# PoseLib/PoseLib

Measured on AMD Instinct MI355X. Metric: scored RANSAC hypotheses/sec (P3P@5k corrs, 5pt@5k corrs), higher is better.
Workload: dtype f64; 1 GPU; p3p_5000; correspondences=5000, problems_in_flight_per_gpu=128, distinct_scenes=64

## Files before the change

include/poselib_amd.h:

```cpp
#ifndef POSELIB_AMD_H_
#define POSELIB_AMD_H_
#include <stddef.h>
#include <stdint.h>

#ifdef __cplusplus
extern "C" {
#endif

#define PL_OK 0
#define PL_ERR_NO_DEVICE (-1)
#define PL_ERR_HIP (-2)
#define PL_ERR_INVALID (-3)
#define PL_ERR_UNSUPPORTED (-4)
#define PL_ERR_COMM (-5)

typedef struct {
    uint64_t max_iterations;
    uint64_t min_iterations;
    double dyn_num_trials_mult;
    double success_prob;
    uint64_t seed;
    int32_t progressive_sampling;
    int32_t score_initial_model;
    uint64_t max_prosac_iterations;
// ... 123 lines not shown
} pl_batch_item;
int pl_estimate_batch(pl_batch_item *items, size_t count, int max_in_flight);
int pl_estimate_batch_devices(pl_batch_item *items, size_t count, const int *devices, int num_devices, int max_in_flight);
typedef struct {
    int32_t kind;
    int32_t status;
    pl_device_points a;
    pl_device_points b;
    size_t n;
    const pl_robust_options *opt;
    pl_camera *camera1;
    const pl_camera *camera2;
    void *model;
    uint8_t *inliers;
    pl_ransac_stats *stats;
} pl_batch_item_dev;
int pl_estimate_batch_dev(pl_batch_item_dev *items, size_t count, int max_in_flight);
int pl_debug_point_stats_group_dev(const pl_device_points *x1, const pl_device_points *x2, const size_t *n, size_t count, int centroid,
                                   double *out);
typedef struct {
    const void *data;
    int64_t stride;
    int32_t dtype;
    int32_t reserved;
    double min_score;
} pl_device_scores;
int pl_estimate_dev_scored(int kind, const pl_device_points *a, const pl_device_points *b, const pl_device_scores *scores, size_t n,
                           const pl_robust_options *opt, pl_camera *camera1, const pl_camera *camera2, void *model, uint8_t *inliers,
                           pl_ransac_stats *stats, size_t *n_used);
int pl_estimate_batch_dev_scored(pl_batch_item_dev *items, const pl_device_scores *scores, size_t *n_used, size_t count,
                                 int max_in_flight);
typedef struct {
    uint8_t *data;
    int64_t stride;
} pl_device_mask;
int pl_estimate_dev_masked(int kind, const pl_device_points *a, const pl_device_points *b, const pl_device_scores *scores ,
                           size_t n, const pl_robust_options *opt, pl_camera *camera1, const pl_camera *camera2, void *model,
                           const pl_device_mask *mask, pl_ransac_stats *stats, size_t *n_used);
int pl_estimate_batch_dev_masked(pl_batch_item_dev *items, const pl_device_scores *scores , const pl_device_mask *masks,
                                 size_t *n_used, size_t count, int max_in_flight);
int pl_debug_rank_scores(const pl_device_scores *scores, const size_t *n, size_t count, uint32_t *order, size_t *kept);
int pl_debug_rank_tile(size_t max_n);
typedef struct {
    uint64_t items;
    uint64_t grouped;
    uint64_t focal_grouped;
    uint64_t solo;
    uint64_t fallback;
} pl_batch_report;
void pl_last_batch_report(pl_batch_report *out);

int pl_ransac_pnp(const double *x, const double *X, size_t n, const pl_robust_options *opt, pl_camera_pose *pose,
                  uint8_t *inliers, pl_ransac_stats *stats);
int pl_ransac_pnpf(const double *x, const double *X, size_t n, const pl_robust_options *opt, pl_camera_pose *pose, double *focal,
                   uint8_t *inliers, pl_ransac_stats *stats);
int pl_ransac_relpose(const double *x1, const double *x2, size_t n, const pl_robust_options *opt, pl_camera_pose *pose,
                      uint8_t *inliers, pl_ransac_stats *stats);
int pl_ransac_shared_focal_relpose(const double *x1, const double *x2, size_t n, const pl_robust_options *opt, pl_camera_pose *pose,
                                   double *focal, uint8_t *inliers, pl_ransac_stats *stats);
int pl_refine_shared_focal_relpose(const double *x1, const double *x2, size_t n, const pl_bundle_options *opt, pl_camera_pose *pose,
                                   double *focal, uint32_t *lm_iterations);

int pl_ransac_fundamental(const double *x1, const double *x2, size_t n, const pl_robust_options *opt, double *F,
                          uint8_t *inliers, pl_ransac_stats *stats);
int pl_ransac_homography(const double *x1, const double *x2, size_t n, const pl_robust_options *opt, double *H,
                         uint8_t *inliers, pl_ransac_stats *stats);
int pl_estimate_1D_radial_absolute_pose(const double *points2D, const double *points3D, size_t n, const pl_robust_options *opt,
                                        pl_camera_pose *pose, uint8_t *inliers, pl_ransac_stats *stats);
int pl_ransac_1D_radial_pnp(const double *x, const double *X, size_t n, const pl_robust_options *opt, pl_camera_pose *pose,
                            uint8_t *inliers, pl_ransac_stats *stats);

typedef struct pl_problem pl_problem;
int pl_problem_create(int kind, const double *a, const double *b, size_t n, pl_problem **out);
int pl_problem_create_tangent(const double *x1, const double *x2, size_t n, const pl_camera *camera1, const pl_camera *camera2,
                              pl_problem **out);
int pl_problem_create_dev(int kind, const pl_device_points *a, const pl_device_points *b, size_t n, pl_problem **out);
int pl_problem_create_tangent_dev(const pl_device_points *x1, const pl_device_points *x2, size_t n, const pl_camera *camera1,
                                  const pl_camera *camera2, pl_problem **out);
void pl_problem_destroy(pl_problem *p);
int pl_ransac_run(pl_problem *p, const pl_robust_options *opt, void *model, uint8_t *inliers, pl_ransac_stats *stats);

typedef struct {
    pl_problem *problem;
    const pl_robust_options *opt;
    void *model;
    uint8_t *inliers;
    pl_ransac_stats *stats;
    int32_t status;
    int32_t reserved;
} pl_ransac_item;
int pl_ransac_batch(pl_ransac_item *items, size_t count, int max_in_flight, int group_size);

typedef int (*pl_allgather_fn)(void *user, const void *send, void *recv, size_t bytes);
typedef struct pl_shard {
    int32_t rank, world;
    pl_allgather_fn allgather;
    void *user;
} pl_shard;
int pl_ransac_run_sharded(pl_problem *p, const pl_robust_options *opt, const pl_shard *shard, void *model,
                          uint8_t *inliers, pl_ransac_stats *stats);

int pl_score_model(pl_problem *p, const void *model, double max_error, uint64_t *inlier_count, double *score);
int pl_debug_inlier_mask(pl_problem *p, const void *model, double max_error, uint8_t *mask);
int pl_debug_tangent_chunk(void);
int pl_debug_radial1d_chunk(void);
int pl_debug_group_slices(int kind, uint32_t n_points, uint32_t iterations, uint32_t launch_chunks);
int pl_debug_radial1d_generate(pl_problem *p, const uint32_t *samples, size_t num_iters, uint32_t slots_per_iter, double *models,
                               uint32_t *num_models, uint32_t *totals);
int pl_debug_generate(pl_problem *p, const uint32_t *samples, uint64_t seed, uint64_t pos_base, const uint32_t *positions, size_t num_iters,
                      uint32_t slots_per_iter, int real_focal_check, int route, double *models, uint32_t *num_models, uint32_t *nan_bits,
                      uint32_t *blk_tot, uint32_t *blk_nan, uint32_t *flags);
int pl_debug_score_stream(pl_problem *p, const void *models, size_t n, double max_error, uint32_t *counts,
                          double *scores, int32_t *path_used);
int pl_debug_score_shape(int kind, uint32_t n_points, int matrix_core, int group_form, uint32_t *chunks,
                         uint32_t *points_per_lane);
typedef struct pl_debug_score_member {
    pl_problem *problem;
    const void *models;
    size_t n;
    double max_error;
    uint32_t *counts;
    double *scores;
    uint32_t slices;
    uint32_t slices_used;
    uint32_t chunks;
    int32_t path_used;
} pl_debug_score_member;
int pl_debug_score_stream_ex(int route, pl_debug_score_member *members, size_t num_members, uint32_t *idle_changed);
typedef struct pl_debug_prune_member {
    pl_problem *problem;
    const void *models;
    size_t n;
    double max_error;
    double init_min;
    uint32_t init_max;
    uint32_t cand_cap;
    uint32_t *counts;
    double *scores;
    uint8_t *kept;
    uint32_t *cand;
    uint32_t num_cand;
    uint32_t cstar, chunks, chunk_points;
    uint32_t lead;
    uint32_t lead_max;
    uint32_t num_live, num_selected;
    uint32_t slices, num_preselected;
    double lead_min;
} pl_debug_prune_member;
int pl_debug_score_pruned(int route, pl_debug_prune_member *members, size_t num_members, uint32_t *idle_changed);
int pl_debug_score_survivors(int route, pl_debug_prune_member *members, size_t num_members, uint32_t *const *survivors,
                             uint32_t *idle_changed, uint32_t *guard_changed);
int pl_debug_score_bounded(int route, pl_debug_prune_member *members, size_t num_members, uint32_t *const *bound_counts,
                           double *const *bound_scores, uint8_t *const *tiers, uint32_t *idle_changed, uint32_t *guard_changed);
int pl_debug_score_prune_gate(int kind, uint32_t n_points, uint32_t iterations);
int pl_debug_lm_route(int kind, uint32_t n_points, uint64_t max_iterations, uint32_t *slices);
typedef struct pl_debug_sampler_shape_info {
    uint64_t window;
    uint32_t build, tile;
    uint32_t small_flags, small_doubling, small_segments;
    uint32_t large_flags, large_doubling, large_segments;
} pl_debug_sampler_shape_info;
int pl_debug_sampler_shape(int K, uint64_t N, uint32_t B, uint64_t window, pl_debug_sampler_shape_info *out);
typedef struct pl_debug_sampler_member {
    uint64_t seed, pos_base, N;
    uint32_t B, M;
    const uint8_t *planted;
    uint32_t *positions;
    uint8_t *delta;
    uint64_t *flagbits;
    uint64_t pos_after;
    uint32_t orbit_error, M_used, build_used;
    int32_t delta_guard, ctl_clear, pad;
} pl_debug_sampler_member;
int pl_debug_sample_positions(int route, int K, int build, pl_debug_sampler_member *members, size_t num_members, uint32_t *idle_changed);
int pl_debug_device_math(int fn, const double *x, size_t n, double *out);
int pl_debug_device_math2(int fn, const double *x, const double *y, size_t n, double *out);
int pl_refine_model(pl_problem *p, const pl_bundle_options *opt, const pl_camera *camera, const uint8_t *mask,
                    void *model, uint32_t *lm_iterations);

int pl_bundle_adjust_camera(pl_problem *p, const pl_bundle_options *opt, pl_camera *camera, const uint8_t *mask,
                            pl_camera_pose *pose, uint32_t *lm_iterations);

int pl_p3p(const double *x , const double *X , pl_camera_pose *out );
int pl_p5lp_radial(const double *x , const double *X , pl_camera_pose *out , int *count );
int pl_relpose_5pt(const double *x1 , const double *x2 , pl_camera_pose *out );
int pl_essential_matrix_5pt(const double *x1, const double *x2, double *E );
int pl_relpose_7pt(const double *x1 , const double *x2 , double *F );
int pl_homography_4pt(const double *x1 , const double *x2 , double *H );
int pl_p35pf(const double *x, const double *X, pl_camera_pose *out, double *focals);
int pl_relpose_6pt_shared_focal(const double *x1, const double *x2, pl_camera_pose *out, double *focals);
int pl_solve_focal_batch(int kind, const double *in, size_t count, double *out_models, uint32_t *out_counts);
int pl_solve_batch(int kind, const double *in, size_t count, double *out_models, uint32_t *out_counts);

#ifdef __cplusplus
}
#endif
#endif
```

poselib_amd/_lib.py:

```python
from __future__ import annotations

import ctypes as C
import os
import subprocess

_PKG = os.path.dirname(os.path.abspath(__file__))
_CSRC = os.path.join(_PKG, "csrc")
LIB_PATH = os.path.join(_PKG, "lib", "libposelib_amd.so")
if os.environ.get("POSELIB_AMD_LIB"):
    LIB_PATH = os.environ["POSELIB_AMD_LIB"]

u64, i32, u32, f64 = C.c_uint64, C.c_int32, C.c_uint32, C.c_double

PL_OK, PL_ERR_NO_DEVICE, PL_ERR_HIP, PL_ERR_INVALID, PL_ERR_UNSUPPORTED, PL_ERR_COMM = 0, -1, -2, -3, -4, -5


class RansacOptions(C.Structure):
    _fields_ = [("max_iterations", u64), ("min_iterations", u64), ("dyn_num_trials_mult", f64), ("success_prob", f64),
                ("seed", u64), ("progressive_sampling", i32), ("score_initial_model", i32),
                ("max_prosac_iterations", u64)]


class BundleOptions(C.Structure):
    _fields_ = [("max_iterations", u64), ("loss_type", i32), ("lambda_update", i32), ("damping", i32), ("verbose", i32),
# ... 60 lines not shown
                ("lead_max", u32), ("num_live", u32), ("num_selected", u32), ("slices", u32), ("num_preselected", u32), ("lead_min", f64)]


class DebugSamplerShape(C.Structure):
    _fields_ = [("window", u64), ("build", u32), ("tile", u32), ("small_flags", u32), ("small_doubling", u32), ("small_segments", u32),
                ("large_flags", u32), ("large_doubling", u32), ("large_segments", u32)]


class DebugSamplerMember(C.Structure):
    _fields_ = [("seed", u64), ("pos_base", u64), ("N", u64), ("B", u32), ("M", u32), ("planted", C.c_void_p), ("positions", C.c_void_p),
                ("delta", C.c_void_p), ("flagbits", C.c_void_p), ("pos_after", u64), ("orbit_error", u32), ("M_used", u32),
                ("build_used", u32), ("delta_guard", i32), ("ctl_clear", i32), ("pad", i32)]


PL_F64, PL_F32 = 0, 1


class DevicePoints(C.Structure):
    _fields_ = [("data", C.c_void_p), ("row_stride", C.c_int64), ("dtype", i32), ("cols", i32)]


class BatchItemDev(C.Structure):
    _fields_ = [("kind", i32), ("status", i32), ("a", DevicePoints), ("b", DevicePoints), ("n", C.c_size_t),
                ("opt", C.POINTER(RobustOptions)), ("camera1", C.POINTER(Camera)), ("camera2", C.POINTER(Camera)),
                ("model", C.c_void_p), ("inliers", C.c_void_p), ("stats", C.POINTER(RansacStats))]


class DeviceScores(C.Structure):
    _fields_ = [("data", C.c_void_p), ("stride", C.c_int64), ("dtype", i32), ("reserved", i32), ("min_score", f64)]


class DevicePointsOut(C.Structure):
    _fields_ = [("data", C.c_void_p), ("row_stride", C.c_int64), ("dtype", i32), ("cols", i32)]


class UndistortItemDev(C.Structure):
    _fields_ = [("status", i32), ("reserved", i32), ("camera", C.POINTER(Camera)), ("points2D", DevicePoints), ("n", C.c_size_t),
                ("out", DevicePointsOut)]


class DeviceMask(C.Structure):
    _fields_ = [("data", C.c_void_p), ("stride", C.c_int64)]


class PoseLibAmdError(RuntimeError):
    pass


def build(force: bool = False, verbose: bool = False) -> str:
    srcs = [os.path.join(_CSRC, f) for f in os.listdir(_CSRC) if f.endswith((".h", ".hip", ".cc", ".inc", "Makefile"))]
    srcs.append(os.path.join(os.path.dirname(_PKG), "include", "poselib_amd.h"))
    stale = (not os.path.exists(LIB_PATH)) or any(os.path.getmtime(s) > os.path.getmtime(LIB_PATH) for s in srcs)
    if force or stale:
        cmd = ["make", "-C", _CSRC]
        if not verbose:
            cmd.append("-s")
        subprocess.check_call(cmd)
    return LIB_PATH


_lib = None


def lib():
    global _lib
    if _lib is None:
        if not os.path.exists(LIB_PATH):
            raise PoseLibAmdError(
                f"{LIB_PATH} is missing: build it with `python -c 'import poselib_amd; poselib_amd.build()'` "
                "(there is no CPU fallback)")
        if not os.environ.get("POSELIB_AMD_KEEP_ENV"):
            os.environ.setdefault("GPU_MAX_HW_QUEUES", "16")
        L = C.CDLL(LIB_PATH)
        _declare(L)
        _lib = L
    return _lib


def _declare(L):
    vp, sz, dbl, cint = C.c_void_p, C.c_size_t, C.c_double, C.c_int
    P = C.POINTER
    opt, stats, cam, pose = P(RobustOptions), P(RansacStats), P(Camera), P(CameraPose)
    dpts = P(DevicePoints)
    sig = {
        "pl_default_ransac_options": (None, [P(RansacOptions)]),
        "pl_default_bundle_options": (None, [P(BundleOptions)]),
        "pl_default_robust_options": (None, [opt, cint]),
        "pl_device_count": (cint, []),
        "pl_set_lm_mode": (cint, [cint]),
        "pl_set_device": (cint, [cint]),
        "pl_last_error": (C.c_char_p, []),
        "pl_version": (C.c_char_p, []),
        "pl_abi_version": (cint, []),
        "pl_estimate_absolute_pose": (cint, [vp, vp, sz, opt, cam, pose, vp, stats]),
        "pl_estimate_relative_pose": (cint, [vp, vp, sz, cam, cam, opt, pose, vp, stats]),
        "pl_estimate_fundamental": (cint, [vp, vp, sz, opt, vp, vp, stats]),
        "pl_estimate_homography": (cint, [vp, vp, sz, opt, vp, vp, stats]),
        "pl_estimate_absolute_pose_dev": (cint, [dpts, dpts, sz, opt, cam, pose, vp, stats]),
        "pl_estimate_relative_pose_dev": (cint, [dpts, dpts, sz, cam, cam, opt, pose, vp, stats]),
        "pl_estimate_fundamental_dev": (cint, [dpts, dpts, sz, opt, vp, vp, stats]),
        "pl_estimate_homography_dev": (cint, [dpts, dpts, sz, opt, vp, vp, stats]),
        "pl_problem_create_dev": (cint, [cint, dpts, dpts, sz, P(vp)]),
        "pl_problem_create_tangent_dev": (cint, [dpts, dpts, sz, cam, cam, P(vp)]),
        "pl_debug_check_device_points": (cint, [dpts, sz, cint]),
        "pl_debug_point_stats_dev": (cint, [dpts, dpts, sz, cint, vp]),
        "pl_estimate_batch": (cint, [P(BatchItem), sz, cint]),
        "pl_estimate_batch_devices": (cint, [P(BatchItem), sz, P(C.c_int), cint, cint]),
        "pl_estimate_batch_dev": (cint, [P(BatchItemDev), sz, cint]),
        "pl_debug_point_stats_group_dev": (cint, [dpts, dpts, P(sz), sz, cint, vp]),
        "pl_estimate_dev_scored": (cint, [cint, dpts, dpts, P(DeviceScores), sz, opt, cam, cam, vp, vp, stats, P(sz)]),
        "pl_estimate_batch_dev_scored": (cint, [P(BatchItemDev), P(DeviceScores), P(sz), sz, cint]),
        "pl_estimate_dev_masked": (cint, [cint, dpts, dpts, P(DeviceScores), sz, opt, cam, cam, vp, P(DeviceMask), stats, P(sz)]),
        "pl_estimate_batch_dev_masked": (cint, [P(BatchItemDev), P(DeviceScores), P(DeviceMask), P(sz), sz, cint]),
        "pl_debug_rank_scores": (cint, [P(DeviceScores), P(sz), sz, vp, P(sz)]),
        "pl_debug_rank_tile": (cint, [sz]),
        "pl_last_batch_report": (None, [P(BatchReport)]),
        "pl_ransac_batch": (cint, [P(RansacItem), sz, cint, cint]),
        "pl_undistort_points": (cint, [cam, vp, sz, vp]),
        "pl_undistort_points_dev": (cint, [cam, dpts, sz, P(DevicePointsOut)]),
        "pl_undistort_points_batch_dev": (cint, [P(UndistortItemDev), sz]),
        "pl_ransac_pnp": (cint, [vp, vp, sz, opt, pose, vp, stats]),
        "pl_ransac_pnpf": (cint, [vp, vp, sz, opt, pose, P(dbl), vp, stats]),
        "pl_ransac_relpose": (cint, [vp, vp, sz, opt, pose, vp, stats]),
        "pl_ransac_shared_focal_relpose": (cint, [vp, vp, sz, opt, pose, P(dbl), vp, stats]),
        "pl_solve_focal_batch": (cint, [cint, vp, sz, vp, vp]),
        "pl_p35pf": (cint, [vp, vp, vp, vp]),
        "pl_relpose_6pt_shared_focal": (cint, [vp, vp, vp, vp]),
        "pl_refine_shared_focal_relpose": (cint, [vp, vp, sz, P(BundleOptions), pose, P(dbl), P(C.c_uint32)]),
        "pl_estimate_shared_focal_relative_pose": (cint, [vp, vp, sz, vp, opt, pose, P(dbl), vp, stats]),
        "pl_ransac_fundamental": (cint, [vp, vp, sz, opt, vp, vp, stats]),
        "pl_ransac_homography": (cint, [vp, vp, sz, opt, vp, vp, stats]),
        "pl_problem_create": (cint, [cint, vp, vp, sz, P(vp)]),
        "pl_problem_create_tangent": (cint, [vp, vp, sz, cam, cam, P(vp)]),
        "pl_debug_inlier_mask": (cint, [vp, vp, dbl, vp]),
        "pl_debug_tangent_chunk": (cint, []),
        "pl_debug_radial1d_chunk": (cint, []),
        "pl_debug_group_slices": (cint, [cint, C.c_uint32, C.c_uint32, C.c_uint32]),
        "pl_debug_radial1d_generate": (cint, [vp, vp, sz, C.c_uint32, vp, vp, vp]),
        "pl_debug_generate": (cint, [vp, vp, u64, u64, vp, sz, C.c_uint32, cint, cint, vp, vp, vp, vp, vp, vp]),
        "pl_estimate_1D_radial_absolute_pose": (cint, [vp, vp, sz, opt, pose, vp, stats]),
        "pl_ransac_1D_radial_pnp": (cint, [vp, vp, sz, opt, pose, vp, stats]),
        "pl_p5lp_radial": (cint, [vp, vp, P(CameraPose), P(cint)]),
        "pl_problem_destroy": (None, [vp]),
        "pl_ransac_run": (cint, [vp, opt, vp, vp, stats]),
        "pl_ransac_run_sharded": (cint, [vp, opt, P(Shard), vp, vp, stats]),
        "pl_score_model": (cint, [vp, vp, dbl, P(C.c_uint64), P(dbl)]),
        "pl_debug_score_stream": (cint, [vp, vp, sz, dbl, vp, vp, P(C.c_int32)]),
        "pl_debug_score_shape": (cint, [cint, C.c_uint32, cint, cint, P(C.c_uint32), P(C.c_uint32)]),
        "pl_debug_score_stream_ex": (cint, [cint, P(DebugScoreMember), sz, P(C.c_uint32)]),
        "pl_debug_score_pruned": (cint, [cint, P(DebugPruneMember), sz, P(C.c_uint32)]),
        "pl_debug_score_survivors": (cint, [cint, P(DebugPruneMember), sz, P(C.c_void_p), P(C.c_uint32), P(C.c_uint32)]),
        "pl_debug_score_bounded": (cint, [cint, P(DebugPruneMember), sz, P(C.c_void_p), P(C.c_void_p), P(C.c_void_p), P(C.c_uint32),
                                           P(C.c_uint32)]),
        "pl_debug_score_prune_gate": (cint, [cint, C.c_uint32, C.c_uint32]),
        "pl_debug_lm_route": (cint, [cint, C.c_uint32, u64, P(C.c_uint32)]),
        "pl_debug_sampler_shape": (cint, [cint, u64, C.c_uint32, u64, P(DebugSamplerShape)]),
        "pl_debug_sample_positions": (cint, [cint, cint, cint, P(DebugSamplerMember), sz, P(C.c_uint32)]),
        "pl_debug_device_math": (cint, [cint, vp, sz, vp]),
        "pl_debug_device_math2": (cint, [cint, vp, vp, sz, vp]),
        "pl_refine_model": (cint, [vp, P(BundleOptions), cam, vp, vp, P(C.c_uint32)]),
        "pl_bundle_adjust_camera": (cint, [vp, P(BundleOptions), cam, vp, P(CameraPose), P(C.c_uint32)]),
        "pl_p3p": (cint, [vp, vp, P(CameraPose)]),
        "pl_relpose_5pt": (cint, [vp, vp, P(CameraPose)]),
        "pl_essential_matrix_5pt": (cint, [vp, vp, vp]),
        "pl_relpose_7pt": (cint, [vp, vp, vp]),
        "pl_homography_4pt": (cint, [vp, vp, vp]),
        "pl_solve_batch": (cint, [cint, vp, sz, vp, vp]),
    }
    missing = [name for name in EXPORTED_SYMBOLS if name not in sig]
    assert not missing, f"no signature declared for {missing}"
    for name, (res, args) in sig.items():
        fn = getattr(L, name)
        fn.restype = res
        fn.argtypes = args
    if L.pl_abi_version() != ABI_VERSION:
        raise PoseLibAmdError(f"{LIB_PATH} has record layout version {L.pl_abi_version()}, this binding was written for {ABI_VERSION}: rebuild")


def check(rc: int):
    if rc < 0:
        msg = lib().pl_last_error().decode()
        raise PoseLibAmdError(f"poselib_amd error {rc}: {msg}")
    return rc


ABI_VERSION = 5
EXPORTED_SYMBOLS = [
    "pl_default_ransac_options", "pl_default_bundle_options", "pl_default_robust_options", "pl_device_count",
    "pl_set_device", "pl_last_error", "pl_version", "pl_estimate_absolute_pose", "pl_estimate_relative_pose",
    "pl_estimate_fundamental", "pl_estimate_homography", "pl_ransac_pnp", "pl_ransac_relpose", "pl_ransac_fundamental",
    "pl_ransac_homography", "pl_problem_create", "pl_problem_destroy", "pl_ransac_run", "pl_ransac_run_sharded", "pl_score_model", "pl_debug_score_stream", "pl_refine_model", "pl_bundle_adjust_camera", "pl_p3p", "pl_relpose_5pt",
    "pl_essential_matrix_5pt", "pl_relpose_7pt", "pl_homography_4pt", "pl_solve_batch", "pl_estimate_batch", "pl_estimate_batch_devices", "pl_last_batch_report", "pl_undistort_points",
    "pl_ransac_batch", "pl_debug_device_math", "pl_debug_device_math2", "pl_ransac_pnpf", "pl_ransac_shared_focal_relpose", "pl_refine_shared_focal_relpose",
    "pl_estimate_shared_focal_relative_pose", "pl_solve_focal_batch", "pl_p35pf", "pl_relpose_6pt_shared_focal", "pl_set_lm_mode",
    "pl_abi_version", "pl_problem_create_tangent", "pl_debug_inlier_mask", "pl_debug_tangent_chunk",
    "pl_p5lp_radial", "pl_debug_radial1d_chunk", "pl_debug_radial1d_generate", "pl_debug_group_slices", "pl_debug_generate",
    "pl_debug_score_shape", "pl_debug_score_stream_ex", "pl_debug_score_pruned", "pl_debug_score_survivors", "pl_debug_score_prune_gate",
    "pl_debug_score_bounded", "pl_debug_lm_route",
    "pl_estimate_absolute_pose_dev", "pl_estimate_relative_pose_dev", "pl_estimate_fundamental_dev", "pl_estimate_homography_dev",
    "pl_problem_create_dev", "pl_problem_create_tangent_dev", "pl_debug_check_device_points", "pl_debug_point_stats_dev",
    "pl_debug_sampler_shape", "pl_debug_sample_positions", "pl_estimate_batch_dev", "pl_debug_point_stats_group_dev",
    "pl_estimate_dev_scored", "pl_estimate_batch_dev_scored", "pl_debug_rank_scores", "pl_debug_rank_tile",
    "pl_undistort_points_dev", "pl_undistort_points_batch_dev", "pl_estimate_dev_masked", "pl_estimate_batch_dev_masked",
]
```

poselib_amd/api.py:

```python
from __future__ import annotations

import ctypes as C
import math
import sys
import threading

import numpy as np

from . import _lib as L

LAMBDA_UPDATES = {"NIELSEN": 0, "FIXED_FACTOR": 1}
DAMPINGS = {"LEVENBERG": 0, "MARQUARDT": 1}
LOSS_TYPES = {"TRIVIAL": 0, "TRUNCATED": 1, "HUBER": 2, "CAUCHY": 3, "TRUNCATED_CAUCHY": 4, "TRUNCATED_LE_ZACH": 5}
CAMERA_MODEL_IDS = {"NULL": -1, "SIMPLE_PINHOLE": 0, "PINHOLE": 1, "SIMPLE_RADIAL": 2, "RADIAL": 3, "OPENCV": 4,
                    "OPENCV_FISHEYE": 5, "SIMPLE_RADIAL_FISHEYE": 8, "RADIAL_FISHEYE": 9}
_CAMERA_NAMES = {v: k for k, v in CAMERA_MODEL_IDS.items()}
KIND_ABS, KIND_REL, KIND_FUND, KIND_HOM = 0, 1, 2, 3
KIND_SHARED_FOCAL = 4
KIND_RAD1D = 5
_POSE_KINDS = (KIND_ABS, KIND_REL, KIND_RAD1D)


class CameraPose:

# ... 683 lines not shown
                out.append((_pypose(model), _info(st, inl[: pr.n])))
            else:
                out.append((model.reshape(3, 3).T.copy(), _info(st, inl[: pr.n])))
        return out


def device_math(fn: int, x):
    x = np.ascontiguousarray(x, dtype=np.float64)
    out = np.zeros_like(x)
    L.check(L.lib().pl_debug_device_math(int(fn), _ptr(x), C.c_size_t(x.size), _ptr(out)))
    return out


def device_math2(fn: int, x, y=None):
    x = np.ascontiguousarray(x, dtype=np.float64)
    if y is not None:
        y = np.ascontiguousarray(y, dtype=np.float64)
        if y.shape != x.shape:
            raise ValueError("x and y differ in shape")
    out = np.zeros_like(x)
    L.check(L.lib().pl_debug_device_math2(int(fn), _ptr(x), None if y is None else _ptr(y), C.c_size_t(x.size), _ptr(out)))
    return out


def group_slices(kind: int, n_points: int, iterations: int, launch_chunks: int) -> int:
    return L.check(L.lib().pl_debug_group_slices(int(kind), int(n_points), int(iterations), int(launch_chunks)))


def score_shape(kind: int, n_points: int, matrix_core: bool, group_form: bool):
    chunks, per_lane = C.c_uint32(0), C.c_uint32(0)
    rc = L.lib().pl_debug_score_shape(int(kind), int(n_points), int(bool(matrix_core)), int(bool(group_form)), C.byref(chunks),
                                      C.byref(per_lane))
    if rc == L.PL_ERR_UNSUPPORTED:
        return None
    L.check(rc)
    return chunks.value, per_lane.value


def score_stream_group(members):
    arr = (L.DebugScoreMember * max(len(members), 1))()
    keep = []
    for i, (problem, models, max_error, slices) in enumerate(members):
        n, flat = problem._flat_models(models)
        cnt = np.zeros(max(n, 1), dtype=np.uint32)
        sc = np.zeros(max(n, 1), dtype=np.float64)
        keep.append((n, flat, cnt, sc))
        arr[i] = L.DebugScoreMember(problem._h, _ptr(flat), n, float(max_error), _ptr(cnt), _ptr(sc), int(slices), 0, 0, 0)
    idle = C.c_uint32(0)
    L.check(L.lib().pl_debug_score_stream_ex(2, arr, C.c_size_t(len(members)), C.byref(idle)))
    out = [{"counts": cnt[:n], "scores": sc[:n], "path": arr[i].path_used, "slices": arr[i].slices_used, "chunks": arr[i].chunks}
           for i, (n, _, cnt, sc) in enumerate(keep)]
    return out, idle.value


def sampler_shape(K: int, N: int, B: int, window: int = 0):
    s = L.DebugSamplerShape()
    L.check(L.lib().pl_debug_sampler_shape(int(K), int(N), int(B), int(window), C.byref(s)))
    return {"window": int(s.window), "build": "small" if s.build == 1 else "large", "tile": int(s.tile),
            "small": {"flags": s.small_flags, "doubling": s.small_doubling, "segments": s.small_segments},
            "large": {"flags": s.large_flags, "doubling": s.large_doubling, "segments": s.large_segments}}


_SAMPLER_BUILDS = {None: 0, "small": 1, "large": 2}


def sample_positions(K: int, members, build=None, group: bool = False):
    arr = (L.DebugSamplerMember * max(len(members), 1))()
    keep = []
    for i, m in enumerate(members):
        planted = m.get("planted")
        if planted is not None:
            planted = np.ascontiguousarray(planted, dtype=np.uint8)
            M = int(planted.size)
            if m.get("M", 0) not in (0, M):
                raise ValueError("a planted table has M bytes")
        else:
            M = int(m.get("M", 0)) or sampler_shape(K, m["N"], m["B"])["window"]
        pos = np.zeros(max(int(m["B"]), 1), dtype=np.uint32)
        cap = M if M < (1 << 31) else 0
        delta = np.zeros(cap + 1, dtype=np.uint8)
        bits = np.zeros(cap // 64 + 2, dtype=np.uint64)
        keep.append((planted, pos, delta, bits))
        arr[i] = L.DebugSamplerMember(int(m.get("seed", 0)), int(m.get("pos_base", 0)), int(m["N"]), int(m["B"]), M,
                                      None if planted is None else _ptr(planted), _ptr(pos), _ptr(delta), _ptr(bits))
    idle = C.c_uint32(0)
    L.check(L.lib().pl_debug_sample_positions(2 if group else 0, int(K), _SAMPLER_BUILDS[build], arr, C.c_size_t(len(members)),
                                              C.byref(idle)))
    out = []
    for i, (_, pos, delta, bits) in enumerate(keep):
        a = arr[i]
        words = (a.M_used + 63) // 64
        out.append({"positions": pos, "delta": delta[:a.M_used], "flagbits": bits[:words], "guard": bits[words:a.M_used // 64 + 2],
                    "pos_after": int(a.pos_after), "orbit_error": int(a.orbit_error), "M": int(a.M_used),
                    "build": "small" if a.build_used == 1 else "large", "delta_guard": bool(a.delta_guard),
                    "ctl_clear": bool(a.ctl_clear)})
    return out, idle.value


def score_prune_gate(kind: int, n_points: int, iterations: int) -> bool:
    return bool(L.check(L.lib().pl_debug_score_prune_gate(int(kind), int(n_points), int(iterations))))


def lm_route(kind: int, n_points: int, max_iterations: int = 100):
    slices = C.c_uint32(0)
    return L.check(L.lib().pl_debug_lm_route(int(kind), int(n_points), int(max_iterations), C.byref(slices))), slices.value


def score_pruned(members, route=0):
    arr = (L.DebugPruneMember * max(len(members), 1))()
    keep = []
    cap = 4096
    for i, (problem, models, max_error, init_max, init_min) in enumerate(members):
        n, flat = problem._flat_models(models)
        cnt = np.zeros(max(n, 1), dtype=np.uint32)
        sc = np.zeros(max(n, 1), dtype=np.float64)
        kp = np.zeros(max(n, 1), dtype=np.uint8)
        cand = np.zeros(cap, dtype=np.uint32)
        keep.append((n, flat, cnt, sc, kp, cand))
        arr[i] = L.DebugPruneMember(problem._h, _ptr(flat), n, float(max_error), float(init_min), int(init_max), cap, _ptr(cnt),
                                    _ptr(sc), _ptr(kp), _ptr(cand))
    idle = C.c_uint32(0)
    L.check(L.lib().pl_debug_score_pruned(int(route), arr, C.c_size_t(len(members)), C.byref(idle)))
    out = []
    for i, (n, _, cnt, sc, kp, cand) in enumerate(keep):
        a = arr[i]
        out.append({"counts": cnt[:n], "scores": sc[:n], "kept": kp[:n].astype(bool), "cand": cand[:min(a.num_cand, cap)].copy(),
                    "num_cand": a.num_cand, "cstar": a.cstar, "chunks": a.chunks, "chunk_points": a.chunk_points, "lead": a.lead,
                    "lead_max": a.lead_max, "lead_min": a.lead_min, "num_live": a.num_live, "num_selected": a.num_selected, "num_preselected": a.num_preselected,
                    "slices": a.slices})
    return out, idle.value


def score_survivors(members, route=0):
    arr = (L.DebugPruneMember * max(len(members), 1))()
    outs = (C.c_void_p * max(len(members), 1))()
    keep = []
    for i, (problem, models, max_error) in enumerate(members):
        n, flat = problem._flat_models(models)
        chunks = score_shape(problem.kind, problem.n, True, route == 2)[0]
        sv = np.zeros((chunks, max(n, 1)), dtype=np.uint32)
        keep.append((n, flat, sv))
        arr[i] = L.DebugPruneMember(problem._h, _ptr(flat), n, float(max_error))
        outs[i] = sv.ctypes.data
    idle, guard = C.c_uint32(0), C.c_uint32(0)
    L.check(L.lib().pl_debug_score_survivors(int(route), arr, C.c_size_t(len(members)), outs, C.byref(idle), C.byref(guard)))
    out = []
    for i, (n, _, sv) in enumerate(keep):
        a = arr[i]
        assert a.chunks == sv.shape[0], (a.chunks, sv.shape)
        out.append({"survivors": sv[:, :n], "chunks": a.chunks, "chunk_points": a.chunk_points, "num_live": a.num_live, "slices": a.slices})
    return out, idle.value, guard.value


def score_bounded(members, route=0):
    arr = (L.DebugPruneMember * max(len(members), 1))()
    bcs, bss, trs = ((C.c_void_p * max(len(members), 1))() for _ in range(3))
    keep = []
    cap = 4096
    for i, (problem, models, max_error, init_max, init_min) in enumerate(members):
        n, flat = problem._flat_models(models)
        cnt = np.zeros(max(n, 1), dtype=np.uint32)
        sc = np.zeros(max(n, 1), dtype=np.float64)
        kp = np.zeros(max(n, 1), dtype=np.uint8)
        cand = np.zeros(cap, dtype=np.uint32)
        bc = np.zeros(max(n, 1), dtype=np.uint32)
        bs = np.zeros(max(n, 1), dtype=np.float64)
        tr = np.zeros(max(n, 1), dtype=np.uint8)
        keep.append((n, flat, cnt, sc, kp, cand, bc, bs, tr))
        arr[i] = L.DebugPruneMember(problem._h, _ptr(flat), n, float(max_error), float(init_min), int(init_max), cap, _ptr(cnt),
                                    _ptr(sc), _ptr(kp), _ptr(cand))
        bcs[i], bss[i], trs[i] = bc.ctypes.data, bs.ctypes.data, tr.ctypes.data
    idle, guard = C.c_uint32(0), C.c_uint32(0)
    L.check(L.lib().pl_debug_score_bounded(int(route), arr, C.c_size_t(len(members)), bcs, bss, trs, C.byref(idle), C.byref(guard)))
    out = []
    for i, (n, _, cnt, sc, kp, cand, bc, bs, tr) in enumerate(keep):
        a = arr[i]
        out.append({"counts": cnt[:n], "scores": sc[:n], "kept": kp[:n].astype(bool), "cand": cand[:min(a.num_cand, cap)].copy(),
                    "num_cand": a.num_cand, "cstar": a.cstar, "chunks": a.chunks, "chunk_points": a.chunk_points, "lead": a.lead,
                    "lead_max": a.lead_max, "lead_min": a.lead_min, "num_live": a.num_live, "num_selected": a.num_selected,
                    "num_preselected": a.num_preselected, "slices": a.slices, "bound_counts": bc[:n], "bound_scores": bs[:n],
                    "tiers": tr[:n]})
    return out, idle.value, guard.value


def ransac_batch(problems, opts, max_in_flight=4, group_size=16):
    b = RansacBatch(problems, opts)
    b.run(max_in_flight, group_size)
    return b.results()


def estimate_fundamental(points2D_1, points2D_2, opt=None, initial_F=None, scores=None, min_score=None, inliers_out=None):
    return _estimate_matrix("pl_estimate_fundamental", KIND_FUND, points2D_1, points2D_2, opt, initial_F, scores, min_score, inliers_out)


def estimate_homography(points2D_1, points2D_2, opt=None, initial_H=None, scores=None, min_score=None, inliers_out=None):
    return _estimate_matrix("pl_estimate_homography", KIND_HOM, points2D_1, points2D_2, opt, initial_H, scores, min_score, inliers_out)


def _ransac(fn, kind, a, b, dim_b, opt, initial):
    a, b = _pts(a, 2), _pts(b, dim_b)
    o = _robust_options(opt, kind, initial is not None)
    n = a.shape[0]
    inl = np.zeros(max(n, 1), dtype=np.uint8)
    st = L.RansacStats()
    if kind in _POSE_KINDS:
        pose = _cpose(initial if initial is not None else CameraPose())
        L.check(getattr(L.lib(), fn)(_ptr(a), _ptr(b), C.c_size_t(n), C.byref(o), C.byref(pose), _ptr(inl), C.byref(st)))
        return _pypose(pose), _info(st, inl[:n])
    M = np.ascontiguousarray((np.eye(3) if initial is None else np.asarray(initial, dtype=np.float64)).T.reshape(9))
    L.check(getattr(L.lib(), fn)(_ptr(a), _ptr(b), C.c_size_t(n), C.byref(o), _ptr(M), _ptr(inl), C.byref(st)))
    return M.reshape(3, 3).T.copy(), _info(st, inl[:n])


def ransac_pnp(x, X, opt=None, initial_pose=None):
    return _ransac("pl_ransac_pnp", KIND_ABS, x, X, 3, opt, initial_pose)


def ransac_1D_radial_pnp(x, X, opt=None, initial_pose=None):
    return _ransac("pl_ransac_1D_radial_pnp", KIND_RAD1D, x, X, 3, opt, initial_pose)


def estimate_1D_radial_absolute_pose(points2D, points3D, opt=None, initial_pose=None):
    return _ransac("pl_estimate_1D_radial_absolute_pose", KIND_RAD1D, points2D, points3D, 3, opt, initial_pose)


def ransac_pnpf(x, X, opt=None):
    x, X = _pts(x, 2), _pts(X, 3)
    o = _robust_options(opt, KIND_ABS, False)
    n = x.shape[0]
    inl = np.zeros(max(n, 1), dtype=np.uint8)
    st = L.RansacStats()
    pose = _cpose(CameraPose())
    focal = C.c_double(1.0)
    L.check(L.lib().pl_ransac_pnpf(_ptr(x), _ptr(X), C.c_size_t(n), C.byref(o), C.byref(pose), C.byref(focal), _ptr(inl), C.byref(st)))
    return Image(_pypose(pose), Camera("SIMPLE_PINHOLE", [focal.value, 0.0, 0.0])), _info(st, inl[:n])


class ImagePair:

    def __init__(self, pose=None, camera1=None, camera2=None):
        self.pose = pose or CameraPose()
        self.camera1 = camera1 or Camera("SIMPLE_PINHOLE", [1.0, 0.0, 0.0])
        self.camera2 = camera2 or Camera("SIMPLE_PINHOLE", list(self.camera1.params))


def _shared_focal_pair(pose, focal, pp):
    return ImagePair(_pypose(pose), Camera("SIMPLE_PINHOLE", [focal, pp[0], pp[1]]), Camera("SIMPLE_PINHOLE", [focal, pp[0], pp[1]]))


def ransac_shared_focal_relpose(x1, x2, opt=None, initial_pair=None):
    x1, x2 = _pts(x1, 2), _pts(x2, 2)
    o = _robust_options(opt, KIND_REL, initial_pair is not None)
    n = x1.shape[0]
    inl = np.zeros(max(n, 1), dtype=np.uint8)
    st = L.RansacStats()
    pose = _cpose(initial_pair.pose if initial_pair is not None else CameraPose())
    focal = C.c_double(initial_pair.camera1.focal() if initial_pair is not None else 1.0)
    L.check(L.lib().pl_ransac_shared_focal_relpose(_ptr(x1), _ptr(x2), C.c_size_t(n), C.byref(o), C.byref(pose), C.byref(focal),
                                                   _ptr(inl), C.byref(st)))
    return _shared_focal_pair(pose, focal.value, (0.0, 0.0)), _info(st, inl[:n])


def estimate_shared_focal_relative_pose(points2D_1, points2D_2, pp, opt=None, initial_pair=None):
    x1, x2 = _pts(points2D_1, 2), _pts(points2D_2, 2)
    o = _robust_options(opt, KIND_REL, initial_pair is not None)
    n = x1.shape[0]
    inl = np.zeros(max(n, 1), dtype=np.uint8)
    st = L.RansacStats()
    pose = _cpose(initial_pair.pose if initial_pair is not None else CameraPose())
    focal = C.c_double(initial_pair.camera1.focal() if initial_pair is not None else 1.0)
    ppa = np.ascontiguousarray(pp, dtype=np.float64)
    L.check(L.lib().pl_estimate_shared_focal_relative_pose(_ptr(x1), _ptr(x2), C.c_size_t(n), _ptr(ppa), C.byref(o), C.byref(pose),
                                                           C.byref(focal), _ptr(inl), C.byref(st)))
    return _shared_focal_pair(pose, focal.value, ppa), _info(st, inl[:n])


def refine_shared_focal_relpose(x1, x2, pair, bundle=None):
    x1, x2 = _pts(x1, 2), _pts(x2, 2)
    o = _robust_options({"bundle": bundle or {}}, KIND_REL, False)
    pose = _cpose(pair.pose)
    focal = C.c_double(pair.camera1.focal())
    its = C.c_uint32(0)
    L.check(L.lib().pl_refine_shared_focal_relpose(_ptr(x1), _ptr(x2), C.c_size_t(x1.shape[0]), C.byref(o.bundle), C.byref(pose),
                                                   C.byref(focal), C.byref(its)))
    return _shared_focal_pair(pose, focal.value, (0.0, 0.0)), its.value


def solve_focal_batch(kind, inputs):
    k = {"p35pf": 0, "relpose_6pt_shared_focal": 1}[kind]
    a = np.ascontiguousarray(inputs, dtype=np.float64)
    per, slots = (20, 10) if k == 0 else (36, 60)
    if a.ndim != 2 or a.shape[1] != per:
        raise ValueError(f"expected a (count, {per}) array")
    models = np.zeros((a.shape[0], slots, 8))
    counts = np.zeros(max(a.shape[0], 1), dtype=np.uint32)
    L.check(L.lib().pl_solve_focal_batch(C.c_int(k), _ptr(a), C.c_size_t(a.shape[0]), _ptr(models), _ptr(counts)))
    return models, counts[: a.shape[0]]


def p35pf(x, X):
    models, counts = solve_focal_batch("p35pf", np.r_[_pts(x, 2).reshape(-1), _pts(X, 3).reshape(-1)][None, :])
    return [(CameraPose(m[:4], m[4:7]), float(m[7])) for m in models[0, : counts[0]]]


def relpose_6pt_shared_focal(x1, x2):
    models, counts = solve_focal_batch("relpose_6pt_shared_focal", np.r_[_pts(x1, 3).reshape(-1), _pts(x2, 3).reshape(-1)][None, :])
    return [(CameraPose(m[:4], m[4:7]), float(m[7])) for m in models[0, : counts[0]]]


def ransac_relpose(x1, x2, opt=None, initial_pose=None):
    return _ransac("pl_ransac_relpose", KIND_REL, x1, x2, 2, opt, initial_pose)


def ransac_fundamental(x1, x2, opt=None, initial_F=None):
    return _ransac("pl_ransac_fundamental", KIND_FUND, x1, x2, 2, opt, initial_F)


def ransac_homography(x1, x2, opt=None, initial_H=None):
    return _ransac("pl_ransac_homography", KIND_HOM, x1, x2, 2, opt, initial_H)


class Problem:

    def __init__(self, kind: int, a, b):
        self.kind = kind
        pts = _Points(a, b, 2, 3 if kind in (KIND_ABS, KIND_RAD1D) else 2)
        self.n = pts.n
        self._h = C.c_void_p()
        L.check(pts.fn("pl_problem_create")(kind, pts.a, pts.b, C.c_size_t(self.n), C.byref(self._h)))

    def run(self, opt=None, initial=None):
        o = _robust_options(opt, self.kind, initial is not None)
        inl = np.zeros(max(self.n, 1), dtype=np.uint8)
        st = L.RansacStats()
# ... 413 lines not shown
```

poselib_amd/csrc/driver.cc:

```cpp
#include "../../include/poselib_amd.h"
#include "pl_focal.h"
#include "pl_kernels.h"
#include "pl_ranges.h"
#include "pl_refine_cam.h"
#include "pl_sfocal.h"
#include "pl_solver_6ptf.h"
#include "pl_solver_p35pf.h"
#include "pl_sampler.h"
#include "pl_svd3.h"

#include <algorithm>
#include <atomic>
#include <chrono>
#include <condition_variable>
#include <cmath>
#include <cstdio>
#include <cstdlib>
#include <cstring>
#include <functional>
#include <limits>
#include <mutex>
#include <string>
#include <thread>
#include <vector>
// ... 2453 lines not shown
        return rc;
    bb.nan_bits = nullptr;
    GroupArgs a;
    wire_batch_step(a, run, s, bb);
    rc = debug_score_prepare(c, p, a, bb, z, recs, ident, H);
    if (rc != PL_OK)
        return rc;
    const int path = a.comp.s16.out ? 2 : (run.pf.enabled ? 1 : 0);
    const uint32_t per = (uint32_t)kStreamWaves * 64u / (uint32_t)kScoreThreads;
    const uint32_t slices = slices_in ? slices_in * per : std::max<uint32_t>(1u, std::min<uint32_t>(1536u / s.chunks, H));
    HIP_TRY(launch_score(p->kind, a.score, slices, c->stream));
    HIP_TRY(launch_finalize(a.rec.f, c->stream));
    if (counts)
        HIP_TRY(hipMemcpyAsync(counts, c->count.p, sizeof(uint32_t) * H, hipMemcpyDeviceToHost, c->stream));
    if (scores)
        HIP_TRY(hipMemcpyAsync(scores, c->score.p, sizeof(double) * H, hipMemcpyDeviceToHost, c->stream));
    HIP_TRY(wait_stream(c));
    if (path_used)
        *path_used = path;
    if (slices_used)
        *slices_used = std::max<uint32_t>(1u, slices / per);
    if (chunks_used)
        *chunks_used = chunks;
    return PL_OK;
}
constexpr size_t kDebugScoreMembers = 4;
int debug_score_group(pl_debug_score_member *m, size_t count, uint32_t *idle_changed) {
    if (!m || count == 0 || count > kDebugScoreMembers)
        return fail(PL_ERR_INVALID, "the group form takes 1 .. 4 members");
    for (size_t i = 0; i < count; ++i) {
        if (!m[i].problem || !m[i].models || m[i].n == 0 || m[i].n > (1u << 22) || m[i].problem->n == 0)
            return fail(PL_ERR_INVALID, "member: problem / models missing, no correspondences, or n outside 1 .. 2^22");
        if (m[i].problem->kind != m[0].problem->kind)
            return fail(PL_ERR_INVALID, "the members of a group are of one kind");
    }
    const int kind = m[0].problem->kind;
    if (kind != EST_ABS && kind != EST_REL && kind != EST_FUND && kind != EST_HOM)
        return fail(PL_ERR_INVALID, "tangent and 1D-radial problems have no group form");
    Context *c;
    int rc = get_context(&c);
    if (rc != PL_OK)
        return rc;
    for (size_t i = 0; i < count; ++i)
        if (m[i].problem->device != c->device)
            return fail(PL_ERR_INVALID, "problem lives on another device than the calling thread's");
    struct Slot {
        BatchRun run{};
        BatchShape s{};
        BatchSizes z{};
        BatchBuffers b{};
        size_t bytes = 0;
        char *arena = nullptr;
        ~Slot() {
            if (arena)
                (void)hipFree(arena);
        }
    } slot[1 + kDebugScoreMembers];
    struct Scratch {
        void *p = nullptr;
        ~Scratch() {
            if (p)
                (void)hipFree(p);
        }
    } dtable;
    GroupArgs ha[1 + kDebugScoreMembers];
    GroupDims dims{};
    dims.G = (uint32_t)count + 1;
    dims.P = group_points_per_lane(kind);
    uint32_t launch_chunks = 0;
    for (size_t i = 0; i < count; ++i) {
        Slot &t = slot[i + 1];
        const pl_problem *p = m[i].problem;
        t.run.kind = kind;
        t.run.pts = p->ps;
        t.run.thr2 = m[i].max_error * m[i].max_error;
        t.run.pf = problem_prefilter(p, t.run.thr2);
        t.run.init_max = 0xffffffffu;
        t.s.Bl = (uint32_t)m[i].n, t.s.slots = 1;
        t.s.use_mfma = score_uses_mfma(kind, p->n, t.run.pf);
        t.s.chunks = group_member_chunks(kind, t.s.use_mfma, p->n);
        t.s.point_rows = t.s.chunks * 64u * (uint32_t)dims.P;
        if (m[i].slices > score_slice_limit(kind, t.s.chunks, false))
            return fail(PL_ERR_INVALID, "slices beyond what the scorer's launch takes for this member");
        t.z = batch_step_sizes(kind, t.s);
        if (t.s.use_mfma)
            launch_chunks += t.s.chunks;
    }
    slot[0].run = slot[1].run, slot[0].s = slot[1].s, slot[0].z = slot[1].z;
    for (size_t k = 0; k <= count; ++k) {
        Slot &t = slot[k];
        BatchBuffers unused;
        t.bytes = pack_batch_buffers(nullptr, t.z, unused);
        HIP_TRY(hipMalloc((void **)&t.arena, t.bytes));
        HIP_TRY(hipMemsetAsync(t.arena, k == 0 ? 0xa5 : 0, t.bytes, c->stream));
        pack_batch_buffers(t.arena, t.z, t.b);
        t.b.nan_bits = nullptr;
        t.b.host_meta = nullptr, t.b.host_models = nullptr, t.b.host_ctl = nullptr;
        wire_batch_step(ha[k], t.run, t.s, t.b);
    }
    ha[0].active = 0;
    for (size_t i = 0; i < count; ++i) {
        GroupArgs &a = ha[i + 1];
        const Slot &t = slot[i + 1];
        const uint32_t H = t.s.Bl;
        a.slices = m[i].slices ? m[i].slices
                               : group_score_slices(kind, t.s.use_mfma, group_expected_hypotheses(kind, H, H), H, t.s.chunks, launch_chunks);
        dims.max_B = std::max(dims.max_B, H);
        dims.max_hcap = std::max(dims.max_hcap, a.score.hyp_capacity);
        dims.max_chunks = std::max(dims.max_chunks, a.chunks);
        dims.max_slices = std::max(dims.max_slices, a.slices);
        dims.any_mfma |= a.use_mfma;
        dims.any_queue |= a.use_mfma ? 0u : 1u;
        std::vector<double> recs;
        std::vector<uint32_t> ident(H);
        for (uint32_t k = 0; k < H; ++k)
            ident[k] = k;
        debug_score_records(m[i].problem, m[i].models, H, recs);
        rc = debug_score_prepare(c, m[i].problem, a, t.b, t.z, recs, ident, H);
        if (rc != PL_OK)
            return rc;
        HIP_TRY(hipStreamSynchronize(c->stream));
    }
    ha[0].slices = ha[1].slices;
    HIP_TRY(hipMalloc(&dtable.p, sizeof(GroupArgs) * dims.G));
    HIP_TRY(hipMemcpyAsync(dtable.p, ha, sizeof(GroupArgs) * dims.G, hipMemcpyHostToDevice, c->stream));
    HIP_TRY(launch_group_score(kind, static_cast<const GroupArgs *>(dtable.p), dims, c->stream));
    HIP_TRY(launch_group_finalize_records(static_cast<const GroupArgs *>(dtable.p), dims, c->stream));
    for (size_t i = 0; i < count; ++i) {
        const Slot &t = slot[i + 1];
        if (m[i].counts)
            HIP_TRY(hipMemcpyAsync(m[i].counts, t.b.count, sizeof(uint32_t) * t.s.Bl, hipMemcpyDeviceToHost, c->stream));
        if (m[i].scores)
            HIP_TRY(hipMemcpyAsync(m[i].scores, t.b.score, sizeof(double) * t.s.Bl, hipMemcpyDeviceToHost, c->stream));
    }
    std::vector<uint32_t> idle(slot[0].bytes / 4);
    HIP_TRY(hipMemcpyAsync(idle.data(), slot[0].arena, idle.size() * 4, hipMemcpyDeviceToHost, c->stream));
    HIP_TRY(wait_stream(c));
    uint32_t changed = 0;
    for (uint32_t w : idle)
        changed += w != 0xa5a5a5a5u ? 1u : 0u;
    if (idle_changed)
        *idle_changed = changed;
    for (size_t i = 0; i < count; ++i) {
        m[i].path_used = ha[i + 1].comp.s16.out ? 2 : (slot[i + 1].run.pf.enabled ? 1 : 0);
        m[i].slices_used = ha[i + 1].slices;
        m[i].chunks = ha[i + 1].chunks;
    }
    return PL_OK;
}
struct DebugBoundedOut {
    uint32_t *const *bound_counts;
    double *const *bound_scores;
    uint8_t *const *tiers;
};
int debug_score_pruned(int route, pl_debug_prune_member *m, size_t count, uint32_t *idle_changed, uint32_t *const *survivors = nullptr,
                       uint32_t *guard_changed = nullptr, const DebugBoundedOut *bounded = nullptr) {
    if (route != 0 && route != 2)
        return fail(PL_ERR_INVALID, "route: 0 single launch, 2 group form");
    if (!m || count == 0 || count > (route == 0 ? 1 : kDebugScoreMembers))
        return fail(PL_ERR_INVALID, "the single launch takes one member, the group form 1 .. 4");
    for (size_t i = 0; i < count; ++i) {
        if (!m[i].problem || !m[i].models || m[i].n == 0 || m[i].n > (1u << 22) || m[i].problem->n == 0)
            return fail(PL_ERR_INVALID, "member: problem / models missing, no correspondences, or n outside 1 .. 2^22");
        if (m[i].problem->kind != EST_ABS)
            return fail(PL_ERR_INVALID, "the pruned scorer is the absolute-pose one");
        if (m[i].cand_cap && !m[i].cand)
            return fail(PL_ERR_INVALID, "member: cand_cap without cand");
    }
    Context *c;
    int rc = get_context(&c);
    if (rc != PL_OK)
        return rc;
    for (size_t i = 0; i < count; ++i)
        if (m[i].problem->device != c->device)
            return fail(PL_ERR_INVALID, "problem lives on another device than the calling thread's");
    struct Slot {
        BatchRun run{};
        BatchShape s{};
        BatchSizes z{};
        BatchBuffers b{};
        size_t bytes = 0;
        char *arena = nullptr;
        ~Slot() {
            if (arena)
                (void)hipFree(arena);
        }
    } slot[1 + kDebugScoreMembers];
    struct Scratch {
        void *p = nullptr;
        ~Scratch() {
            if (p)
                (void)hipFree(p);
        }
    } dtable, dbound[kDebugScoreMembers];
    GroupArgs ha[1 + kDebugScoreMembers];
    GroupDims dims{};
    dims.G = (uint32_t)count + 1;
    dims.P = group_points_per_lane(EST_ABS);
    uint32_t launch_chunks = 0;
    for (size_t i = 0; i < count; ++i) {
        Slot &t = slot[i + 1];
        const pl_problem *p = m[i].problem;
        t.run.kind = EST_ABS;
        t.run.pts = p->ps;
        t.run.thr2 = m[i].max_error * m[i].max_error;
        t.run.pf = problem_prefilter(p, t.run.thr2);
        t.run.init_max = m[i].init_max;
        t.run.init_min = m[i].init_min;
        t.s.Bl = (uint32_t)m[i].n, t.s.slots = 1;
        t.s.use_mfma = score_uses_mfma(EST_ABS, p->n, t.run.pf);
        if (!t.s.use_mfma)
            return fail(PL_ERR_UNSUPPORTED, "member: not scored on the matrix cores (size, threshold or coordinates out of range)");
        if (route == 0) {
            t.s.chunks = score_chunks(EST_ABS, p->n, true, true);
            t.s.point_rows = abs16_point_rows(p->n);
        } else {
            t.s.chunks = group_member_chunks(EST_ABS, true, p->n);
            t.s.point_rows = t.s.chunks * 64u * (uint32_t)dims.P;
        }
        t.s.prune = true;
        t.z = batch_step_sizes(EST_ABS, t.s);
        launch_chunks += t.s.chunks;
    }
    slot[0].run = slot[1].run, slot[0].s = slot[1].s, slot[0].z = slot[1].z;
    for (size_t k = (route == 0 ? 1 : 0); k <= count; ++k) {
        Slot &t = slot[k];
        BatchBuffers unused;
        t.bytes = pack_batch_buffers(nullptr, t.z, unused);
        HIP_TRY(hipMalloc((void **)&t.arena, t.bytes));
        HIP_TRY(hipMemsetAsync(t.arena, k == 0 ? 0xa5 : 0, t.bytes, c->stream));
        pack_batch_buffers(t.arena, t.z, t.b);
        t.b.nan_bits = nullptr;
        t.b.host_meta = nullptr, t.b.host_models = nullptr, t.b.host_ctl = nullptr;
        wire_batch_step(ha[k], t.run, t.s, t.b);
        ha[k].score.prune.bound = bounded ? 1u : 0u;
        if (bounded && k > 0) {
            const size_t hcap = ha[k].score.hyp_capacity;
            HIP_TRY(hipMalloc(&dbound[k - 1].p, hcap * 16));
            HIP_TRY(hipMemsetAsync(dbound[k - 1].p, 0xff, hcap * 16, c->stream));
            ha[k].score.prune.bnd_score = static_cast<double *>(dbound[k - 1].p);
            ha[k].score.prune.bnd_count = reinterpret_cast<uint32_t *>(ha[k].score.prune.bnd_score + hcap);
        }
    }
    ha[0].active = 0;
    for (size_t i = 0; i < count; ++i) {
        GroupArgs &a = ha[i + 1];
        const Slot &t = slot[i + 1];
        const uint32_t H = t.s.Bl;
        a.slices = group_score_slices(EST_ABS, true, group_expected_hypotheses(EST_ABS, H, H), H, t.s.chunks, launch_chunks);
        dims.max_B = std::max(dims.max_B, H);
        dims.max_hcap = std::max(dims.max_hcap, a.score.hyp_capacity);
        dims.max_chunks = std::max(dims.max_chunks, a.chunks);
        dims.max_slices = std::max(dims.max_slices, a.slices);
        dims.any_mfma = dims.any_prune = 1;
        dims.any_bound = bounded ? 1u : 0u;
        std::vector<double> recs;
        std::vector<uint32_t> ident(H);
        for (uint32_t k = 0; k < H; ++k)
            ident[k] = k;
        debug_score_records(m[i].problem, m[i].models, H, recs);
        rc = debug_score_prepare(c, m[i].problem, a, t.b, t.z, recs, ident, H);
        if (rc != PL_OK)
            return rc;
        HIP_TRY(hipStreamSynchronize(c->stream));
    }
    uint32_t single_slices = 0;
    if (route == 0) {
        const GroupArgs &a = ha[1];
        const uint32_t slices = std::max<uint32_t>(1u, std::min<uint32_t>(1536u / a.chunks, a.score.hyp_capacity));
        single_slices = std::max<uint32_t>(1u, std::min<uint32_t>(slices * (uint32_t)kScoreThreads / (64u * (uint32_t)kStreamWaves),
                                                                  score_slice_limit(EST_ABS, a.chunks, true)));
        if (survivors) {
            HIP_TRY(launch_score_count(a.score, slices, c->stream));
        } else {
            HIP_TRY(launch_score_pruned(a.score, slices, c->stream));
            if (!bounded)
                HIP_TRY(launch_prune_label(a.score, c->stream));
            HIP_TRY(launch_finalize_records(a.rec, c->stream));
        }
    } else {
        ha[0].slices = ha[1].slices;
        HIP_TRY(hipMalloc(&dtable.p, sizeof(GroupArgs) * dims.G));
        HIP_TRY(hipMemcpyAsync(dtable.p, ha, sizeof(GroupArgs) * dims.G, hipMemcpyHostToDevice, c->stream));
        if (survivors) {
            HIP_TRY(launch_group_score_count(static_cast<const GroupArgs *>(dtable.p), dims, c->stream));
        } else {
            HIP_TRY(launch_group_score(EST_ABS, static_cast<const GroupArgs *>(dtable.p), dims, c->stream));
            for (size_t i = 0; i < count && !bounded; ++i)
                HIP_TRY(launch_prune_label(ha[i + 1].score, c->stream));
            HIP_TRY(launch_group_finalize_records(static_cast<const GroupArgs *>(dtable.p), dims, c->stream));
        }
    }
    std::vector<std::vector<uint32_t>> part(count);
    std::vector<std::vector<uint32_t>> rank(count);
    std::vector<std::vector<uint8_t>> kept(count);
    std::vector<std::vector<RecordMeta>> meta(count);
    std::vector<PruneState> st(count);
    std::vector<BatchCtl> ctl(count);
    std::vector<std::vector<uint32_t>> bcount(count);
    std::vector<std::vector<double>> bscore(count);
    for (size_t i = 0; i < count; ++i) {
        const Slot &t = slot[i + 1];
        const uint32_t H = t.s.Bl;
        if (bounded) {
            const size_t hcap = ha[i + 1].score.hyp_capacity;
            bcount[i].resize(hcap), bscore[i].resize(hcap);
            HIP_TRY(hipMemcpyAsync(bcount[i].data(), ha[i + 1].score.prune.bnd_count, 4 * hcap, hipMemcpyDeviceToHost, c->stream));
            HIP_TRY(hipMemcpyAsync(bscore[i].data(), ha[i + 1].score.prune.bnd_score, 8 * hcap, hipMemcpyDeviceToHost, c->stream));
        }
        if (m[i].counts && !survivors)
            HIP_TRY(hipMemcpyAsync(m[i].counts, t.b.count, sizeof(uint32_t) * H, hipMemcpyDeviceToHost, c->stream));
        if (m[i].scores && !survivors)
            HIP_TRY(hipMemcpyAsync(m[i].scores, t.b.score, sizeof(double) * H, hipMemcpyDeviceToHost, c->stream));
        rank[i].resize(H), kept[i].resize(H), meta[i].resize(kRecordCap);
        HIP_TRY(hipMemcpyAsync(rank[i].data(), t.b.rank, sizeof(uint32_t) * H, hipMemcpyDeviceToHost, c->stream));
        HIP_TRY(hipMemcpyAsync(kept[i].data(), t.b.prune_kept, H, hipMemcpyDeviceToHost, c->stream));
        HIP_TRY(hipMemcpyAsync(meta[i].data(), t.b.rec_meta, sizeof(RecordMeta) * kRecordCap, hipMemcpyDeviceToHost, c->stream));
        HIP_TRY(hipMemcpyAsync(&st[i], t.b.prune_state, sizeof(PruneState), hipMemcpyDeviceToHost, c->stream));
        HIP_TRY(hipMemcpyAsync(&ctl[i], t.b.ctl, sizeof(BatchCtl), hipMemcpyDeviceToHost, c->stream));
        if (survivors || bounded) {
            part[i].resize((size_t)t.s.chunks * ha[i + 1].score.hyp_capacity);
            HIP_TRY(hipMemcpyAsync(part[i].data(), t.b.part_count, sizeof(uint32_t) * part[i].size(), hipMemcpyDeviceToHost, c->stream));
        }
    }
    std::vector<uint32_t> idle(route == 2 ? slot[0].bytes / 4 : 0);
    if (!idle.empty())
        HIP_TRY(hipMemcpyAsync(idle.data(), slot[0].arena, idle.size() * 4, hipMemcpyDeviceToHost, c->stream));
    HIP_TRY(wait_stream(c));
    uint32_t changed = 0;
    for (uint32_t w : idle)
        changed += w != 0xa5a5a5a5u ? 1u : 0u;
    if (idle_changed)
        *idle_changed = changed;
    uint32_t guard = 0;
    for (size_t i = 0; i < count; ++i) {
        const uint32_t H = slot[i + 1].s.Bl, chunks = slot[i + 1].s.chunks;
        m[i].chunks = chunks;
        m[i].chunk_points = slot[i + 1].s.point_rows / chunks;
        m[i].num_live = ctl[i].num_live;
        m[i].slices = route == 0 ? single_slices : ha[i + 1].slices;
        if (survivors) {
            const uint32_t hcap = ha[i + 1].score.hyp_capacity;
            for (uint32_t ch = 0; ch < chunks; ++ch) {
                for (uint32_t k = 0; k < H; ++k)
                    survivors[i][(size_t)ch * H + k] = rank[i][k] == kNoRank ? 0u : part[i][(size_t)ch * hcap + rank[i][k]];
                for (uint32_t p = ctl[i].num_live; p < hcap; ++p)
                    guard += part[i][(size_t)ch * hcap + p] != 0xffffffffu ? 1u : 0u;
            }
            continue;
        }
        if (bounded) {
            const uint32_t hcap = ha[i + 1].score.hyp_capacity;
            for (uint32_t ch = 0; ch < chunks; ++ch)
                for (uint32_t p = ctl[i].num_live; p < hcap; ++p)
                    guard += part[i][(size_t)ch * hcap + p] != 0xffffffffu ? 1u : 0u;
            for (uint32_t k = 0; k < H; ++k) {
                const uint32_t p = rank[i][k];
                const bool live = p != kNoRank;
                const bool has = live && bcount[i][p] != 0xffffffffu;
                bounded->bound_counts[i][k] = has ? bcount[i][p] : 0xffffffffu;
                bounded->bound_scores[i][k] = has ? bscore[i][p] : std::numeric_limits<double>::quiet_NaN();
                bounded->tiers[i][k] = !live ? 3 : kept[i][p] == kKept ? 0 : has ? 2 : 1;
            }
        }
        const bool split = st[i].cstar < chunks;
        uint32_t selected = 0;
        for (uint32_t k = 0; k < H; ++k) {
            const bool live = rank[i][k] != kNoRank;
            const bool kp = !split || !live || kept[i][rank[i][k]] == kKept;
            selected += (split && live && kp) ? 1u : 0u;
            if (m[i].kept)
                m[i].kept[k] = kp ? 1 : 0;
        }
        m[i].num_cand = ctl[i].num_records;
        for (uint32_t r = 0; r < std::min<uint32_t>({ctl[i].num_records, m[i].cand_cap, kRecordCap}); ++r)
            m[i].cand[r] = meta[i][r].k;
        m[i].cstar = st[i].cstar;
        m[i].lead = kPruneLead;
        m[i].lead_max = st[i].lead_max;
        m[i].lead_min = st[i].lead_min;
        m[i].num_selected = selected;
        m[i].num_preselected = st[i].sel_len;
    }
    if (guard_changed)
        *guard_changed = guard;
    return PL_OK;
}
}
int pl_debug_score_pruned(int route, pl_debug_prune_member *members, size_t num_members, uint32_t *idle_changed) {
    if (idle_changed)
        *idle_changed = 0;
    return debug_score_pruned(route, members, num_members, idle_changed);
}
int pl_debug_score_survivors(int route, pl_debug_prune_member *members, size_t num_members, uint32_t *const *survivors,
                             uint32_t *idle_changed, uint32_t *guard_changed) {
    if (idle_changed)
        *idle_changed = 0;
    if (guard_changed)
        *guard_changed = 0;
    if (!survivors)
        return fail(PL_ERR_INVALID, "pl_debug_score_survivors: survivors missing");
    for (size_t i = 0; i < num_members; ++i)
        if (!survivors[i])
            return fail(PL_ERR_INVALID, "pl_debug_score_survivors: a member without an output array");
    return debug_score_pruned(route, members, num_members, idle_changed, survivors, guard_changed);
}
int pl_debug_score_bounded(int route, pl_debug_prune_member *members, size_t num_members, uint32_t *const *bound_counts,
                           double *const *bound_scores, uint8_t *const *tiers, uint32_t *idle_changed, uint32_t *guard_changed) {
    if (idle_changed)
        *idle_changed = 0;
    if (guard_changed)
        *guard_changed = 0;
    if (!bound_counts || !bound_scores || !tiers)
        return fail(PL_ERR_INVALID, "pl_debug_score_bounded: output arrays missing");
    for (size_t i = 0; i < num_members; ++i)
        if (!bound_counts[i] || !bound_scores[i] || !tiers[i])
            return fail(PL_ERR_INVALID, "pl_debug_score_bounded: a member without an output array");
    const DebugBoundedOut out{bound_counts, bound_scores, tiers};
    return debug_score_pruned(route, members, num_members, idle_changed, nullptr, guard_changed, &out);
}
int pl_debug_score_prune_gate(int kind, uint32_t n_points, uint32_t iterations) {
    PrefilterArgs pf{};
    pf.enabled = 1;
    pf.g16 = pf.t16 = pf.h16 = 1.0f, pf.thr = 1.0f;
    if (n_points == 0)
        return fail(PL_ERR_INVALID, "pl_debug_score_prune_gate: n_points > 0");
    const bool mfma = score_uses_mfma(kind, n_points, pf);
    return score_prune_gate(kind, mfma, iterations, kind == EST_ABS ? score_chunks(kind, n_points, true, mfma) : 1u) ? 1 : 0;
}
int pl_debug_lm_route(int kind, uint32_t n_points, uint64_t max_iterations, uint32_t *slices) {
    const bool known = kind == EST_ABS || kind == EST_REL || kind == EST_FUND || kind == EST_HOM || kind == EST_RELT || kind == EST_RAD1D;
    if (!known || n_points == 0 || !slices)
        return fail(PL_ERR_INVALID, "pl_debug_lm_route: kind 0 .. 5, n_points > 0, slices pointer");
    const LMRoute r = lm_route(kind, n_points, true, (uint32_t)std::min<uint64_t>(max_iterations, 0xffffffffu));
    *slices = r.slices;
    return r.kernel;
}
int pl_debug_score_stream(pl_problem *p, const void *models, size_t n, double max_error, uint32_t *counts,
                          double *scores, int32_t *path_used) {
    return debug_score_single(p, models, n, max_error, 0, counts, scores, path_used, nullptr, nullptr);
}
int pl_debug_score_stream_ex(int route, pl_debug_score_member *members, size_t num_members, uint32_t *idle_changed) {
    if (idle_changed)
        *idle_changed = 0;
    if (route != 0 && route != 2)
        return fail(PL_ERR_INVALID, "route: 0 single launch, 2 group form");
    if (route == 2)
        return debug_score_group(members, num_members, idle_changed);
    if (!members || num_members != 1)
        return fail(PL_ERR_INVALID, "the single launch takes one member");
    pl_debug_score_member &m = members[0];
    return debug_score_single(m.problem, m.models, m.n, m.max_error, m.slices, m.counts, m.scores, &m.path_used, &m.slices_used, &m.chunks);
}
int pl_debug_score_shape(int kind, uint32_t n_points, int matrix_core, int group_form, uint32_t *chunks, uint32_t *points_per_lane) {
    const bool four = kind == EST_ABS || kind == EST_REL || kind == EST_FUND || kind == EST_HOM;
    if (!(four || kind == EST_RELT || kind == EST_RAD1D) || n_points == 0 || !chunks || !points_per_lane)
        return fail(PL_ERR_INVALID, "pl_debug_score_shape: kind 0 .. 5, n_points > 0, output pointers");
    if (!four && (matrix_core || group_form))
        return fail(PL_ERR_INVALID, "tangent and 1D-radial problems have neither a matrix-core nor a group form");
    if (matrix_core) {
        PrefilterArgs pf{};
        pf.enabled = 1;
        pf.g16 = pf.t16 = pf.h16 = 1.0f, pf.thr = 1.0f;
        if (!score_uses_mfma(kind, n_points, pf))
            return fail(PL_ERR_UNSUPPORTED, "no problem of this kind and size is scored on the matrix cores");
    }
    if (group_form) {
        *chunks = group_member_chunks(kind, matrix_core != 0, n_points);
        *points_per_lane = (uint32_t)((matrix_core && (kind == EST_REL || kind == EST_FUND)) ? group_mfma2_points_per_lane(kind)
                                                                                           : group_points_per_lane(kind));
    } else {
        *chunks = score_chunks(kind, n_points, true, matrix_core != 0);
        *points_per_lane = (uint32_t)score_points_per_lane(kind, n_points, true, matrix_core != 0);
    }
    return PL_OK;
}

int pl_debug_sampler_shape(int K, uint64_t N, uint32_t B, uint64_t window, pl_debug_sampler_shape_info *out) {
    if ((K != 3 && K != 4 && K != 5 && K != 7) || N < (uint64_t)K || N > 0xffffffffull || B == 0 || !out)
        return fail(PL_ERR_INVALID, "pl_debug_sampler_shape: K in {3, 4, 5, 7}, K <= N < 2^32, B > 0, output pointer");
    const uint64_t M = window ? window : sampler_window((uint32_t)N, K, B);
    const OrbitShape sm = orbit_build_shape(true), lg = orbit_build_shape(false);
    out->window = M;
    out->build = (M <= 0xffffffffull && orbit_small_build((uint32_t)M, N, K)) ? 1u : 2u;
    out->tile = sm.tile;
    out->small_flags = sm.flags, out->small_doubling = sm.doubling, out->small_segments = sm.segments;
    out->large_flags = lg.flags, out->large_doubling = lg.doubling, out->large_segments = lg.segments;
    return PL_OK;
}
int pl_debug_sample_positions(int route, int K, int build, pl_debug_sampler_member *m, size_t count, uint32_t *idle_changed) {
    if (idle_changed)
        *idle_changed = 0;
    if (route != 0 && route != 2)
        return fail(PL_ERR_INVALID, "route: 0 single launches, 2 group form");
    if (build < 0 || build > 2)
        return fail(PL_ERR_INVALID, "build: 0 the launcher's choice, 1 small, 2 large");
    if (K != 3 && K != 4 && K != 5 && K != 7)
        return fail(PL_ERR_INVALID, "K: 3, 4, 5 or 7");
    constexpr size_t kMembers = 4;
    if (!m || count == 0 || count > kMembers)
        return fail(PL_ERR_INVALID, "1 .. 4 members");
    const int kind = K == 3 ? EST_ABS : K == 5 ? EST_REL : K == 7 ? EST_FUND : EST_HOM;
    uint64_t window[kMembers];
    for (size_t i = 0; i < count; ++i) {
        if (m[i].N < (uint64_t)K || m[i].N > 0xffffffffull || m[i].B == 0 || m[i].B > (1u << 20) || !m[i].positions)
            return fail(PL_ERR_INVALID, "member: K <= N < 2^32, B in 1 .. 2^20, positions");
        window[i] = m[i].M ? m[i].M : sampler_window((uint32_t)m[i].N, K, m[i].B);
        if (window[i] > 0x7fffffffull || m[i].pos_base + window[i] >= 0xffffffffull || m[i].pos_base >= 0xffffffffull)
            return fail(PL_ERR_INVALID, "member: a window beyond 2^31 - 1 positions, or one that ends at or beyond draw 2^32 - 1");
        if (route == 2 && (m[i].planted != nullptr) != (m[0].planted != nullptr))
            return fail(PL_ERR_INVALID, "a group is drawn or planted as a whole");
    }
    Context *c;
    int rc = get_context(&c);
    if (rc != PL_OK)
        return rc;
    struct Slot {
        BatchRun run{};
        BatchShape s{};
        BatchSizes z{};
        BatchBuffers b{};
        size_t bytes = 0;
        char *arena = nullptr;
        ~Slot() {
            if (arena)
                (void)hipFree(arena);
        }
    } slot[1 + kMembers];
    struct Scratch {
        void *p = nullptr;
        ~Scratch() {
            if (p)
                (void)hipFree(p);
        }
    } dtable;
    GroupArgs ha[1 + kMembers];
    GroupDims dims{};
    dims.G = (uint32_t)count + 1;
    dims.min_n = 0xffffffffu;
    for (size_t i = 0; i < count; ++i) {
        Slot &t = slot[i + 1];
        t.run.kind = kind;
        t.run.pts.n = (uint32_t)m[i].N;
        t.run.seed = m[i].seed, t.run.pos = m[i].pos_base;
        t.s.B = t.s.Bl = m[i].B, t.s.M = (uint32_t)window[i], t.s.slots = 1, t.s.chunks = 1;
        const BatchSizes full = batch_step_sizes(kind, t.s);
        t.z.positions = full.positions, t.z.delta = full.delta, t.z.flags = full.flags, t.z.ctl = full.ctl;
    }
    slot[0].run = slot[1].run, slot[0].s = slot[1].s, slot[0].z = slot[1].z;
    std::vector<uint64_t> bits;
    for (size_t k = (route == 0 ? 1 : 0); k <= count; ++k) {
        Slot &t = slot[k];
        BatchBuffers unused;
        t.bytes = pack_batch_buffers(nullptr, t.z, unused);
        t.bytes += 256;
        HIP_TRY(hipMalloc((void **)&t.arena, t.bytes));
        HIP_TRY(hipMemsetAsync(t.arena, 0xa5, t.bytes, c->stream));
        pack_batch_buffers(t.arena, t.z, t.b);
        t.b.host_meta = nullptr, t.b.host_models = nullptr, t.b.host_ctl = nullptr;
        wire_batch_step(ha[k], t.run, t.s, t.b);
        if (k == 0)
            continue;
        const pl_debug_sampler_member &mi = m[k - 1];
        group_dims_sampler(dims, t.s.M, t.run.pts.n, t.s.B);
        HIP_TRY(hipMemsetAsync(t.b.positions, 0xff, t.z.positions, c->stream));
        if (mi.planted) {
            const uint32_t M = t.s.M, words = (M + 63u) / 64u;
            bits.assign(words, 0ull);
            for (uint32_t p = 0; p < M; ++p)
                if (mi.planted[p] != (uint8_t)K)
                    bits[p >> 6] |= 1ull << (p & 63u);
// ... 963 lines not shown
```

poselib_amd/csrc/kernels.hip:

```cpp
#include "pl_kernels.h"
#include "pl_global.h"
#include "pl_lm_chain.inc"
#include "pl_device.h"
#include <atomic>
#include "pl_prefilter.h"
#include <cstdlib>
#include "pl_sampler.h"
#include "pl_solver_h4.h"
#include "pl_solver_p3p.h"
#include "pl_solver_p5lp_radial.h"
#include "pl_solver_rel.h"

namespace pl {

typedef const float __attribute__((address_space(4))) *uniform_f32_ptr;
typedef const double __attribute__((address_space(4))) *uniform_f64_ptr;
typedef const uint32_t __attribute__((address_space(4))) *uniform_u32_ptr;
__device__ __forceinline__ uniform_f32_ptr as_uniform(const float *p) { return (uniform_f32_ptr)(uintptr_t)p; }
__device__ __forceinline__ uniform_f64_ptr as_uniform(const double *p) { return (uniform_f64_ptr)(uintptr_t)p; }
__device__ __forceinline__ uniform_u32_ptr as_uniform(const uint32_t *p) { return (uniform_u32_ptr)(uintptr_t)p; }

__device__ __forceinline__ double wave_sum(double v) {
#pragma unroll
    for (int off = 32; off > 0; off >>= 1)
// ... 1043 lines not shown

constexpr int kMfmaQueueCap = 1024;
template <int EST>
__device__ __forceinline__ void mfma_drain(const uint16_t *queue, uint32_t first, uint32_t n0, uint32_t n1, const double *pts, int npw,
                                       const double *__restrict__ models, uint32_t unit_slots, double thr2, double *acc_s,
                                       uint32_t *acc_c) {
    const int lane = threadIdx.x & 63;
    struct Batch {
        uint32_t g;
        bool act;
        double x[EST == EST_ABS ? 5 : 4];
        double M[kModelDoubles];
    };
    auto fetch = [&](uint32_t n, uint32_t at, Batch &b) {
        b.act = (uint32_t)lane < n;
        const uint32_t e = b.act ? (uint32_t)queue[(at + lane) & (kMfmaQueueCap - 1)] : 0xffffu;
        const uint32_t pi = b.act ? (e & 0x1ffu) : 0u;
        b.g = e >> 9;
#pragma unroll
        for (int d = 0; d < (EST == EST_ABS ? 5 : 4); ++d)
            b.x[d] = pts[d * npw + pi];
        const uint32_t slot_g = (uint32_t)__shfl((int)unit_slots, (int)(b.act ? b.g : 0u), 64);
        const double *Mp = models + (size_t)slot_g * kModelStride;
#pragma unroll
        for (int i = 0; i < kModelDoubles; ++i)
            b.M[i] = Mp[i];
    };
    auto finish = [&](const Batch &b) {
        double r2;
        const bool in = eval_point<EST>(b.M, b.x, thr2, r2) && b.act;
        const double v = in ? r2 : 0.0;
        const uint64_t inmask = __builtin_amdgcn_ballot_w64(in);
        const uint32_t g0 = (uint32_t)__builtin_amdgcn_readfirstlane((int)b.g);
        if (inmask && !__builtin_amdgcn_ballot_w64(b.act && b.g != g0)) {
            const double tot = wave_sum_dpp(v);
            if (lane == 0) {
                acc_s[g0] += tot;
                acc_c[g0] += (uint32_t)__popcll(inmask);
            }
        } else if (inmask) {
            add_run_totals(v, inmask, b.g, b.act, lane, acc_s, acc_c);
        }
    };
    __builtin_amdgcn_fence(__ATOMIC_ACQ_REL, "wavefront");
    Batch b0, b1;
    fetch(n0, first, b0);
    if (n1) {
        fetch(n1, first + n0, b1);
        finish(b0);
        finish(b1);
    } else {
        finish(b0);
    }
}

template <int PG>
__device__ __forceinline__ void abs16_tile_bits(const half8_t (&Aop)[kAbs16Dirs], const uint4 (&s_b)[1 + kAbs16Dirs][PG][32], int col, int half,
                                                uint32_t (&out)[16]) {
#pragma unroll
    for (int v = 0; v < 16; ++v)
        out[v] = 0u;
    const float16_t kZero = {0, 0, 0, 0, 0, 0, 0, 0, 0, 0, 0, 0, 0, 0, 0, 0};
    auto products = [&](int g, float16_t &D0, float16_t &D1, float16_t &D2) {
        half8_t Bop[kAbs16Dirs];
#pragma unroll
        for (int d = 0; d < kAbs16Dirs; ++d) {
            const uint4 braw = s_b[half ? 1 + d : 0][g][col];
            __builtin_memcpy(&Bop[d], &braw, 16);
        }
        D0 = __builtin_amdgcn_mfma_f32_32x32x16_f16(Aop[0], Bop[0], kZero, 0, 0, 0);
        D1 = __builtin_amdgcn_mfma_f32_32x32x16_f16(Aop[1], Bop[1], kZero, 0, 0, 0);
        D2 = __builtin_amdgcn_mfma_f32_32x32x16_f16(Aop[2], Bop[2], kZero, 0, 0, 0);
    };
    float16_t D0, D1, D2;
    products(0, D0, D1, D2);
#pragma unroll 16
    for (int g = 1; g < PG; ++g) {
        uint32_t T[16];
#pragma unroll
        for (int v = 0; v < 16; ++v)
            T[v] = __float_as_uint(D0[v]) | __float_as_uint(D1[v]) | __float_as_uint(D2[v]);
        products(g, D0, D1, D2);
#pragma unroll
        for (int v = 0; v < 16; ++v)
            out[v] = __builtin_amdgcn_alignbit(out[v], T[v], 31);
        __builtin_amdgcn_sched_group_barrier(0x002, 16, 0);
        __builtin_amdgcn_sched_group_barrier(0x100, 3, 0);
        __builtin_amdgcn_sched_group_barrier(0x002, 4, 0);
        __builtin_amdgcn_sched_group_barrier(0x008, 1, 0);
        __builtin_amdgcn_sched_group_barrier(0x002, 4, 0);
        __builtin_amdgcn_sched_group_barrier(0x008, 1, 0);
        __builtin_amdgcn_sched_group_barrier(0x002, 4, 0);
        __builtin_amdgcn_sched_group_barrier(0x008, 1, 0);
        __builtin_amdgcn_sched_group_barrier(0x002, 4, 0);
    }
#pragma unroll
    for (int v = 0; v < 16; ++v) {
        const uint32_t sg = __float_as_uint(D0[v]) | __float_as_uint(D1[v]) | __float_as_uint(D2[v]);
        out[v] = __builtin_amdgcn_alignbit(out[v], sg, 31);
    }
}

template <int PG>
__device__ __forceinline__ uint32_t abs16_tile_count_t(const half8_t (&Aop)[kAbs16Dirs], const uint4 (&s_b)[1 + kAbs16Dirs][PG][32], int col,
                                                       int half) {
    static_assert(PG % 2 == 0, "a word holds the 32 pairs of two point groups");
    const float16_t kZero = {0, 0, 0, 0, 0, 0, 0, 0, 0, 0, 0, 0, 0, 0, 0, 0};
    auto products = [&](int g, float16_t &D0, float16_t &D1, float16_t &D2) {
        half8_t Bop[kAbs16Dirs];
#pragma unroll
        for (int d = 0; d < kAbs16Dirs; ++d) {
            const uint4 braw = s_b[half ? 1 + d : 0][g][col];
            __builtin_memcpy(&Bop[d], &braw, 16);
        }
        D0 = __builtin_amdgcn_mfma_f32_32x32x16_f16(Bop[0], Aop[0], kZero, 0, 0, 0);
        D1 = __builtin_amdgcn_mfma_f32_32x32x16_f16(Bop[1], Aop[1], kZero, 0, 0, 0);
        D2 = __builtin_amdgcn_mfma_f32_32x32x16_f16(Bop[2], Aop[2], kZero, 0, 0, 0);
    };
    uint32_t word = 0u, n = 0u;
    float16_t D0, D1, D2;
    products(0, D0, D1, D2);
#pragma unroll 16
    for (int g = 1; g < PG; ++g) {
        uint32_t T[16];
#pragma unroll
        for (int v = 0; v < 16; ++v)
            T[v] = __float_as_uint(D0[v]) | __float_as_uint(D1[v]) | __float_as_uint(D2[v]);
        products(g, D0, D1, D2);
#pragma unroll
        for (int v = 0; v < 16; ++v)
            word = __builtin_amdgcn_alignbit(word, T[v], 31);
        if ((g - 1) % 2)
            n += (uint32_t)__popc(word);
        __builtin_amdgcn_sched_group_barrier(0x002, 16, 0);
        __builtin_amdgcn_sched_group_barrier(0x100, 3, 0);
        __builtin_amdgcn_sched_group_barrier(0x002, 4, 0);
        __builtin_amdgcn_sched_group_barrier(0x008, 1, 0);
        __builtin_amdgcn_sched_group_barrier(0x002, 4, 0);
        __builtin_amdgcn_sched_group_barrier(0x008, 1, 0);
        __builtin_amdgcn_sched_group_barrier(0x002, 4, 0);
        __builtin_amdgcn_sched_group_barrier(0x008, 1, 0);
        __builtin_amdgcn_sched_group_barrier(0x002, 4, 0);
        __builtin_amdgcn_sched_barrier(0);
    }
#pragma unroll
    for (int v = 0; v < 16; ++v) {
        const uint32_t sg = __float_as_uint(D0[v]) | __float_as_uint(D1[v]) | __float_as_uint(D2[v]);
        word = __builtin_amdgcn_alignbit(word, sg, 31);
    }
    n += (uint32_t)__popc(word);
    return 16u * PG - n;
}

constexpr int kScoreAll = 0, kScoreLead = 1, kScoreSel = 2, kScoreCount = 3, kScoreCountAll = 4;
template <int PG, int MODE = kScoreAll>
__device__ __forceinline__ void score_mfma_body(const PointSet &pts, const uint4 *__restrict__ shadow16,
                                                const uint4 *__restrict__ points16,
                                                const double *__restrict__ models, const uint32_t *__restrict__ slots,
                                                const uint32_t *__restrict__ num_hyp_ptr, uint32_t hyp_capacity,
                                                double thr2, uint32_t *__restrict__ part_count,
                                                double *__restrict__ part_score, uint32_t slice, uint32_t chunk,
                                                uint32_t nslices, const uint32_t *__restrict__ sel = nullptr,
                                                uint32_t lead = 0) {
    constexpr int kWaves = kMfmaThreads / 64;
    constexpr int NPW = 32 * PG;
    __shared__ double s_pts[5][NPW];
    __shared__ uint16_t s_queue[kWaves][kMfmaQueueCap];
    __shared__ double s_acc_s[kWaves][64];
    __shared__ uint32_t s_acc_c[kWaves][64];
    __shared__ uint32_t s_next_unit;
    __shared__ uint4 s_b[1 + kAbs16Dirs][PG][32];
    const int lane = threadIdx.x & 63;
    const int wave = __builtin_amdgcn_readfirstlane((int)(threadIdx.x >> 6));
    const int col = lane & 31, half = lane >> 5;

    const uint32_t H = MODE == kScoreLead ? min(*as_uniform(num_hyp_ptr), lead) : *as_uniform(num_hyp_ptr);
    const uint32_t waves_per_chunk = nslices * kWaves;
    {
        uint32_t kb0, gn0;
        if (!unit_of_ticket<32u>(slice * kWaves, H, waves_per_chunk, kb0, gn0))
            return;
    }

    uint32_t validbits = 0;
#pragma unroll
    for (int g = 0; g < PG; ++g)
        validbits |= (chunk * NPW + g * 32 + col < pts.n) ? (1u << (PG - 1 - g)) : 0u;
    const uint4 *const prow = points16 + (size_t)chunk * NPW * 4;
    for (uint32_t j = threadIdx.x; j < (uint32_t)NPW; j += kMfmaThreads) {
        const uint32_t i = chunk * NPW + j;
        const uint32_t ic = i < pts.n ? i : 0u;
#pragma unroll
        for (int d = 0; d < 5; ++d)
            s_pts[d][j] = pts.a[d][ic];
#pragma unroll
        for (int r = 0; r < 1 + kAbs16Dirs; ++r)
            s_b[r][j >> 5][j & 31] = prow[(size_t)j * 4 + r];
    }
    if (threadIdx.x == 0)
        s_next_unit = 0;
    __syncthreads();

    uint16_t *const queue = s_queue[wave];
    double *const acc_s = s_acc_s[wave];
    uint32_t *const acc_c = s_acc_c[wave];
    auto request_ticket = [&]() -> uint32_t {
        uint32_t t = 0;
        if (lane == 0) {
            const uint32_t k = atomicAdd(&s_next_unit, 1u);
            t = slice * kWaves + (k % kWaves) + (k / kWaves) * waves_per_chunk;
        }
        return t;
    };
    uint32_t ticket = (uint32_t)__builtin_amdgcn_readfirstlane((int)request_ticket());
    uint32_t kb, gn;
    while (unit_of_ticket<32u>(ticket, H, waves_per_chunk, kb, gn)) {
        const uint32_t pending = request_ticket();
        uint32_t unit_pos = 0;
        if constexpr (MODE == kScoreSel)
            unit_pos = sel ? sel[kb + min((uint32_t)lane, gn - 1u)] : kb + min((uint32_t)lane, gn - 1u);
        const uint32_t unit_slots = slots[MODE == kScoreSel ? unit_pos : kb + min((uint32_t)lane, gn - 1u)];
        acc_s[lane] = 0.0;
        acc_c[lane] = 0;
        uint32_t qhead = 0, qtail = 0;

        auto drain_pair = [&](uint32_t n2) {
            mfma_drain<EST_ABS>(queue, qhead, 64u, n2, &s_pts[0][0], NPW, models, unit_slots, thr2, acc_s, acc_c);
            qhead += 64u + n2;
        };
        auto drain = [&](uint32_t n) {
            mfma_drain<EST_ABS>(queue, qhead, n, 0u, &s_pts[0][0], NPW, models, unit_slots, thr2, acc_s, acc_c);
            qhead += n;
        };

        const uint32_t ngroups32 = (gn + 31u) / 32u;
        auto load_a = [&](uint32_t hg, uint4 (&A)[kAbs16Dirs]) {
            const uint4 *row = shadow16 + (size_t)(kb + 32u * hg + (uint32_t)col) * 4;
            if constexpr (MODE == kScoreSel)
                row = shadow16 + (size_t)(uint32_t)__shfl((int)unit_pos, (int)(32u * hg + (uint32_t)col), 64) * 4;
#pragma unroll
            for (int d = 0; d < kAbs16Dirs; ++d)
                A[d] = row[half ? 3 : d];
        };
        uint4 Araw[kAbs16Dirs];
        load_a(0, Araw);
        for (uint32_t hg = 0; hg < ngroups32; ++hg) {
            half8_t Aop[kAbs16Dirs];
#pragma unroll
            for (int d = 0; d < kAbs16Dirs; ++d)
                __builtin_memcpy(&Aop[d], &Araw[d], 16);
            if (hg + 1 < ngroups32)
                load_a(hg + 1, Araw);
            uint32_t out[16];
            abs16_tile_bits<PG>(Aop, s_b, col, half, out);
            const bool partial_group = hg * 32u + 32u > gn;
            auto expand_round = [&](int v, bool check_slot) {
                const uint32_t slot = hg * 32u + 8u * (uint32_t)(v >> 2) + 4u * (uint32_t)half + (uint32_t)(v & 3);
                uint32_t bits = ~out[v] & validbits;
                if (check_slot && slot >= gn)
                    bits = 0u;
                const uint64_t anyb = __builtin_amdgcn_ballot_w64(bits != 0u);
                if (anyb) {
                    const uint32_t cnt = (uint32_t)__popc(bits);
                    if (!__builtin_amdgcn_ballot_w64(cnt > 1u)) {
                        const uint32_t below = __builtin_amdgcn_mbcnt_hi((uint32_t)(anyb >> 32), __builtin_amdgcn_mbcnt_lo((uint32_t)anyb, 0u));
                        if (bits) {
                            const uint32_t g = (uint32_t)(PG - 1 - (31 - __clz((int)bits)));
                            queue[(qtail + below) & (kMfmaQueueCap - 1)] = (uint16_t)((slot << 9) | (g * 32u + (uint32_t)col));
                        }
                        qtail += (uint32_t)__popcll(anyb);
                    } else {
                        const uint32_t incl = wave_scan_u32(cnt);
                        const uint32_t total = (uint32_t)__builtin_amdgcn_readlane((int)incl, 63);
                        uint32_t pos = qtail + incl - cnt;
                        uint32_t rest = bits;
                        while (rest) {
                            const int hi = 31 - __clz((int)rest);
                            rest &= ~(1u << hi);
                            const uint32_t g = (uint32_t)(PG - 1 - hi);
                            queue[pos & (kMfmaQueueCap - 1)] = (uint16_t)((slot << 9) | (g * 32u + (uint32_t)col));
                            ++pos;
                        }
                        qtail += total;
                    }
                    while (qtail - qhead >= 128u)
                        drain_pair(64u);
                }
            };
            if (partial_group) {
#pragma unroll
                for (int v = 0; v < 16; ++v)
                    expand_round(v, true);
            } else {
#pragma unroll
                for (int v = 0; v < 16; ++v)
                    expand_round(v, false);
            }
        }
        if (qtail - qhead > 64u)
            drain_pair(qtail - qhead - 64u);
        else if (qtail != qhead)
            drain(qtail - qhead);
        __builtin_amdgcn_fence(__ATOMIC_ACQ_REL, "wavefront");
        if ((uint32_t)lane < gn) {
            const size_t o = MODE == kScoreSel ? (size_t)chunk * hyp_capacity + unit_pos : (size_t)chunk * hyp_capacity + kb + lane;
            part_score[o] = acc_s[lane];
            part_count[o] = acc_c[lane];
        }
        ticket = (uint32_t)__builtin_amdgcn_readfirstlane((int)pending);
    }
}

template <int PG>
__device__ __forceinline__ void score_count_body(uint32_t n_points, const uint4 *__restrict__ shadow16, const uint4 *__restrict__ points16,
                                                 const uint32_t *__restrict__ num_hyp_ptr, uint32_t hyp_capacity,
                                                 uint32_t *__restrict__ survivors, uint32_t slice, uint32_t chunk, uint32_t nslices,
                                                 uint32_t first) {
    constexpr int kWaves = kMfmaThreads / 64;
    constexpr int NPW = 32 * PG;
    __shared__ uint4 s_b[1 + kAbs16Dirs][PG][32];
    __shared__ uint32_t s_next_unit;
    const int lane = threadIdx.x & 63;
    const int col = lane & 31, half = lane >> 5;
    const uint32_t Hall = *as_uniform(num_hyp_ptr);
    if (Hall <= first)
        return;
    const uint32_t H = Hall - first;
    const uint32_t waves_per_chunk = nslices * kWaves;
    {
        uint32_t kb0, gn0;
        if (!unit_of_ticket<32u>(slice * kWaves, H, waves_per_chunk, kb0, gn0))
            return;
    }
    const uint32_t pad = chunk * NPW + NPW > n_points ? chunk * NPW + NPW - n_points : 0u;
    const uint4 *const prow = points16 + (size_t)chunk * NPW * 4;
    for (uint32_t j = threadIdx.x; j < (uint32_t)NPW; j += kMfmaThreads) {
#pragma unroll
        for (int r = 0; r < 1 + kAbs16Dirs; ++r)
            s_b[r][j >> 5][j & 31] = prow[(size_t)j * 4 + r];
    }
    if (threadIdx.x == 0)
        s_next_unit = 0;
    __syncthreads();

    auto request_ticket = [&]() -> uint32_t {
        uint32_t t = 0;
        if (lane == 0) {
            const uint32_t k = atomicAdd(&s_next_unit, 1u);
            t = slice * kWaves + (k % kWaves) + (k / kWaves) * waves_per_chunk;
        }
        return t;
    };
    uint32_t ticket = (uint32_t)__builtin_amdgcn_readfirstlane((int)request_ticket());
    uint32_t kb, gn;
    while (unit_of_ticket<32u>(ticket, H, waves_per_chunk, kb, gn)) {
        const uint32_t pending = request_ticket();
        const uint32_t ngroups32 = (gn + 31u) / 32u;
        auto load_a = [&](uint32_t hg, uint4 (&A)[kAbs16Dirs]) {
            const uint4 *row = shadow16 + (size_t)min(first + kb + 32u * hg + (uint32_t)col, Hall - 1u) * 4;
#pragma unroll
            for (int d = 0; d < kAbs16Dirs; ++d)
                A[d] = row[half ? 3 : d];
        };
        uint4 Araw[kAbs16Dirs];
        load_a(0, Araw);
        for (uint32_t hg = 0; hg < ngroups32; ++hg) {
            half8_t Aop[kAbs16Dirs];
#pragma unroll
            for (int d = 0; d < kAbs16Dirs; ++d)
                __builtin_memcpy(&Aop[d], &Araw[d], 16);
            if (hg + 1 < ngroups32)
                load_a(hg + 1, Araw);
            const uint32_t mine = abs16_tile_count_t<PG>(Aop, s_b, col, half);
            const auto both = __builtin_amdgcn_permlane32_swap(mine, mine, false, false);
            uint32_t total = both[0] + both[1];
            if (pad)
                total = max(total, pad) - pad;
            if (half == 0 && 32u * hg + (uint32_t)col < gn)
                survivors[(size_t)chunk * hyp_capacity + first + kb + 32u * hg + (uint32_t)col] = total;
        }
        ticket = (uint32_t)__builtin_amdgcn_readfirstlane((int)pending);
    }
}

template <int PG>
__global__ __launch_bounds__(kMfmaThreads) __attribute__((amdgpu_waves_per_eu(4, 8))) void k_score_mfma(PointSet pts, const uint4 *__restrict__ shadow16,
                                                               const uint4 *__restrict__ points16,
                                                               const double *__restrict__ models,
                                                               const uint32_t *__restrict__ slots,
                                                               const uint32_t *__restrict__ num_hyp_ptr,
                                                               uint32_t hyp_capacity, double thr2,
                                                               uint32_t *__restrict__ part_count,
                                                               double *__restrict__ part_score,
                                                               uint32_t *__restrict__ tickets) {
    (void)tickets;
    uint32_t slice, chunk;
    slice_chunk_of_workgroup(gridDim.x, gridDim.y, slice, chunk);
    score_mfma_body<PG>(pts, shadow16, points16, models, slots, num_hyp_ptr, hyp_capacity, thr2, part_count, part_score, slice,
                        chunk, gridDim.x);
}
template <int PG>
__global__ __launch_bounds__(kMfmaThreads) __attribute__((amdgpu_waves_per_eu(4, 8))) void k_score_mfma_g(const GroupArgs *ga) {
    const GroupArgs &g = ga[blockIdx.z];
    uint32_t slice, chunk;
    if (!g.active || !g.use_mfma || !slice_chunk_of_workgroup(g.slices, g.chunks, slice, chunk))
        return;
    const ScoreArgs a = globalised(g.score);
    score_mfma_body<PG>(a.pts, static_cast<const uint4 *>(a.shadow16), static_cast<const uint4 *>(a.points16), a.models, a.slots,
                        a.num_hyp, a.hyp_capacity, a.thr2, a.part_count, a.part_score, slice, chunk, g.slices);
}
template <int MODE> __host__ __device__ constexpr uint32_t pruned_slices(uint32_t slices) {
    return MODE == kScoreLead ? (slices < 2u ? slices : 2u) : MODE == kScoreSel ? (slices + 3u) / 4u : slices;
}
template <int PG, int MODE> __device__ __forceinline__ void score_mfma_pruned(const ScoreArgs &a, uint32_t slice, uint32_t chunk, uint32_t nslices) {
    static_assert(MODE == kScoreLead || MODE == kScoreSel || MODE == kScoreCount || MODE == kScoreCountAll, "the plain launch is k_score_mfma's");
    const PruneArgs &pr = a.prune;
    if (!pr.st && MODE != kScoreSel)
        return;
    if constexpr (MODE == kScoreCountAll) {
        score_count_body<PG>(a.pts.n, static_cast<const uint4 *>(a.shadow16), static_cast<const uint4 *>(a.points16), a.num_hyp,
                             a.hyp_capacity, a.part_count, slice, chunk, nslices, 0u);
    } else if constexpr (MODE == kScoreCount) {
        const uint32_t cstar = *as_uniform(&pr.st->cstar);
        if (cstar >= pr.chunks || chunk >= cstar)
            return;
        score_count_body<PG>(a.pts.n, static_cast<const uint4 *>(a.shadow16), static_cast<const uint4 *>(a.points16), a.num_hyp,
                             a.hyp_capacity, a.part_count, slice, chunk, nslices, pr.lead);
    } else {
        const uint32_t *len = MODE == kScoreSel && pr.st ? &pr.st->sel_len : a.num_hyp;
        score_mfma_body<PG, MODE>(a.pts, static_cast<const uint4 *>(a.shadow16), static_cast<const uint4 *>(a.points16), a.models, a.slots,
                                  len, a.hyp_capacity, a.thr2, a.part_count, a.part_score, slice, chunk, nslices, pr.st ? pr.sel : nullptr,
                                  pr.lead);
    }
}
template <int PG, int MODE>
__global__ __launch_bounds__(kMfmaThreads) __attribute__((amdgpu_waves_per_eu(4, 8))) void k_score_mfma_pr(ScoreArgs a) {
    uint32_t slice, chunk;
    slice_chunk_of_workgroup(gridDim.x, gridDim.y, slice, chunk);
    score_mfma_pruned<PG, MODE>(a, slice, chunk, gridDim.x);
}
template <int PG, int MODE>
__global__ __launch_bounds__(kMfmaThreads) __attribute__((amdgpu_waves_per_eu(4, 8))) void k_score_mfma_pr_g(const GroupArgs *ga) {
    const GroupArgs &g = ga[blockIdx.z];
    uint32_t slice, chunk;
    const uint32_t ns = pruned_slices<MODE>(g.slices);
    if (!g.active || !g.use_mfma || !slice_chunk_of_workgroup(ns, g.chunks, slice, chunk))
        return;
    score_mfma_pruned<PG, MODE>(globalised(g.score), slice, chunk, ns);
}

__device__ __forceinline__ void prune_lead_body(const ScoreArgs &a) {
    __shared__ uint32_t wmax[4];
    __shared__ double wmin[4];
    const PruneArgs &pr = a.prune;
    const uint32_t n = min(*a.num_hyp, pr.lead), N = a.pts.n;
    uint32_t bmax = 0;
    double bmin = 1.7976931348623157e308;
    for (uint32_t p = threadIdx.x; p < n; p += 256) {
        uint32_t c = 0;
        double s = 0.0;
        for (uint32_t ch = 0; ch < pr.chunks; ++ch) {
            c += a.part_count[(size_t)ch * a.hyp_capacity + p];
            s += a.part_score[(size_t)ch * a.hyp_capacity + p];
        }
        bmax = max(bmax, c);
        bmin = fmin(bmin, s + (double)(N - c) * a.thr2);
    }
#pragma unroll
    for (int off = 32; off > 0; off >>= 1) {
        bmax = max(bmax, (uint32_t)__shfl_xor(bmax, off, 64));
        bmin = fmin(bmin, __shfl_xor(bmin, off, 64));
    }
    if ((threadIdx.x & 63) == 0) {
        wmax[threadIdx.x >> 6] = bmax;
        wmin[threadIdx.x >> 6] = bmin;
    }
    __syncthreads();
    if (threadIdx.x == 0) {
        uint32_t lmax = pr.init_max;
        double lmin = pr.init_min;
        for (int w = 0; w < 4; ++w) {
            lmax = max(lmax, wmax[w]);
            lmin = fmin(lmin, wmin[w]);
        }
        const double need = fmax(lmin / a.thr2, (double)(N - min(lmax, N))) + (double)kPruneMargin;
        uint32_t cstar = pr.chunks;
        if (need < (double)N)
            cstar = (uint32_t)ceil(need / (double)pr.chunk_points);
        pr.st->lead_max = lmax;
        pr.st->lead_min = lmin;
        pr.st->cstar = max(1u, min(cstar, pr.chunks));
        pr.st->sel_len = 0;
        pr.st->pad = 0;
    }
}
__global__ __launch_bounds__(256) void k_prune_lead(ScoreArgs a) { prune_lead_body(a); }
__global__ __launch_bounds__(256) void k_prune_lead_g(const GroupArgs *ga) {
    const GroupArgs &g = ga[blockIdx.z];
    if (!g.active || !g.use_mfma || !g.score.prune.st)
        return;
    prune_lead_body(globalised(g.score));
}

__device__ __forceinline__ bool prune_rule(uint32_t cs, double sum, uint32_t S, uint32_t N, double thr2, const PruneState &st) {
    return cs + (N - S) <= st.lead_max && sum + (double)(S - cs) * thr2 > st.lead_min * (1.0 + kPruneScoreMargin);
}
__device__ __forceinline__ uint32_t prune_keeps(const ScoreArgs &a, uint32_t p, uint32_t H, uint32_t cstar) {
    const PruneArgs &pr = a.prune;
    if (p >= H)
        return 0u;
    if (p < pr.lead || cstar >= pr.chunks)
        return 1u;
    const uint32_t N = a.pts.n, S = min(cstar * pr.chunk_points, N);
    uint32_t cs = 0;
    for (uint32_t ch = 0; ch < cstar; ++ch)
        cs += a.part_count[(size_t)ch * a.hyp_capacity + p];
    return prune_rule(cs, 0.0, S, N, a.thr2, *pr.st) ? 0u : 1u;
}
__global__ __launch_bounds__(256) void k_prune_label(ScoreArgs a) {
    const PruneArgs &pr = a.prune;
    const uint32_t H = *a.num_hyp, cstar = pr.st->cstar, p = blockIdx.x * 256u + threadIdx.x;
    if (p >= H || p < pr.lead || cstar >= pr.chunks || pr.kept[p] != kKept)
        return;
    const uint32_t N = a.pts.n, S = min(cstar * pr.chunk_points, N);
    uint32_t cs = 0;
    double sum = 0.0;
    for (uint32_t ch = 0; ch < cstar; ++ch) {
        cs += a.part_count[(size_t)ch * a.hyp_capacity + p];
        sum += a.part_score[(size_t)ch * a.hyp_capacity + p];
    }
    if (prune_rule(cs, sum, S, N, a.thr2, *pr.st))
        pr.kept[p] = kPrunedExact;
}
__device__ __forceinline__ void prune_flags_body(const ScoreArgs &a) {
    __shared__ uint32_t wt[16];
    const PruneArgs &pr = a.prune;
    const uint32_t H = *a.num_hyp, cstar = pr.st->cstar;
    if (blockIdx.x * 1024u >= H)
        return;
    const uint32_t p = blockIdx.x * 1024u + threadIdx.x;
    const uint32_t keep = prune_keeps(a, p, H, cstar);
    if (p < H)
        pr.kept[p] = (uint8_t)keep;
    const uint32_t tot = wave_sum_u32(keep);
    if ((threadIdx.x & 63) == 0)
        wt[threadIdx.x >> 6] = tot;
    __syncthreads();
    if (threadIdx.x == 0) {
        uint32_t t = 0;
        for (int w = 0; w < 16; ++w)
            t += wt[w];
        pr.blk_kept[blockIdx.x] = t;
    }
}
__device__ __forceinline__ void prune_list_body(const ScoreArgs &a) {
    __shared__ uint32_t wt[16], wb[16];
    const PruneArgs &pr = a.prune;
    const uint32_t H = *a.num_hyp;
    if (blockIdx.x * 1024u >= H)
        return;
    const int lane = threadIdx.x & 63, wave = threadIdx.x >> 6;
    uint32_t before = 0;
    for (uint32_t j = threadIdx.x; j < blockIdx.x; j += 1024u)
        before += pr.blk_kept[j];
    before = wave_sum_u32(before);
    const uint32_t p = blockIdx.x * 1024u + threadIdx.x;
    const uint32_t keep = p < H ? (uint32_t)pr.kept[p] : 0u;
    const uint32_t inc = wave_scan_u32(keep);
    if (lane == 63)
        wt[wave] = inc;
    if (lane == 0)
        wb[wave] = before;
    __syncthreads();
    uint32_t at = inc - keep;
    for (int w = 0; w < 16; ++w)
        at += wb[w] + (w < wave ? wt[w] : 0u);
    if (keep)
        pr.sel[at] = p;
    if (p == H - 1u)
        pr.st->sel_len = at + keep;
}
__global__ __launch_bounds__(1024) void k_prune_flags(ScoreArgs a) { prune_flags_body(a); }
__global__ __launch_bounds__(1024) void k_prune_list(ScoreArgs a) { prune_list_body(a); }
__global__ __launch_bounds__(1024) void k_prune_flags_g(const GroupArgs *ga) {
    const GroupArgs &g = ga[blockIdx.z];
    if (!g.active || !g.use_mfma || !g.score.prune.st)
        return;
    prune_flags_body(globalised(g.score));
}
__global__ __launch_bounds__(1024) void k_prune_list_g(const GroupArgs *ga) {
    const GroupArgs &g = ga[blockIdx.z];
    if (!g.active || !g.use_mfma || !g.score.prune.st)
        return;
    prune_list_body(globalised(g.score));
}

constexpr int kBoundThreads = 512;
constexpr uint32_t kBoundGroups = 16;
template <int P> __device__ __forceinline__ void score_bound_body(const ScoreArgs &a, uint32_t wg, uint32_t nwg) {
    constexpr int kWaves = kBoundThreads / 64;
    constexpr uint32_t NPW = 64u * P;
    __shared__ uint32_t s_c[kWaves][64];
    __shared__ uint64_t s_q[kWaves][64];
    __shared__ uint32_t s_und[64];
    __shared__ uint32_t s_nund;
    const PruneArgs &pr = a.prune;
    if (!pr.st || !pr.bound || *as_uniform(&pr.st->cstar) >= pr.chunks)
        return;
    const uint32_t first = min(*as_uniform(a.num_hyp), pr.lead), len = *as_uniform(&pr.st->sel_len);
    if (len <= first || (uint64_t)wg * 64u >= len - first)
        return;
    const int lane = threadIdx.x & 63;
    const int wave = __builtin_amdgcn_readfirstlane((int)(threadIdx.x >> 6));
    const PrefilterArgs pf = a.pf;
    const uint32_t chunks = pr.chunks;
    const bool resident = chunks <= (uint32_t)kWaves;
    float x[P], y[P], X[P], Y[P], Z[P], fw[P];
    bool valid[P];
    uint64_t vmask[P];
    auto load_chunk = [&](uint32_t chunk) {
#pragma unroll
        for (int p = 0; p < P; ++p) {
            const uint32_t i = chunk * NPW + (uint32_t)p * 64u + (uint32_t)lane;
            valid[p] = i < a.pts.n;
            vmask[p] = __builtin_amdgcn_ballot_w64(valid[p]);
            const uint32_t ic = valid[p] ? i : 0u;
            const double Xd = a.pts.a[2][ic], Yd = a.pts.a[3][ic], Zd = a.pts.a[4][ic];
            x[p] = (float)a.pts.a[0][ic], y[p] = (float)a.pts.a[1][ic];
            X[p] = (float)Xd, Y[p] = (float)Yd, Z[p] = (float)Zd;
            fw[p] = pf_point_abs(Xd, Yd, Zd, pf.gx);
        }
    };
    load_chunk(min((uint32_t)wave, chunks - 1u));
    const uint32_t lead_max = pr.st->lead_max;
    const double beat = pr.st->lead_min * (1.0 + kPruneScoreMargin);
    auto decide = [&](uint32_t pos) -> bool {
        uint32_t c = 0;
        uint64_t q = 0;
#pragma unroll
        for (int w = 0; w < kWaves; ++w) {
            c += s_c[w][lane];
            q += s_q[w][lane];
        }
        const double qd = (double)q * 9.5367431640625e-07;
        double s_lb = a.thr2 * qd;
        if (fma(a.thr2, qd, -s_lb) < 0.0)
            s_lb = __longlong_as_double(__double_as_longlong(s_lb) - 1);
        const bool keep = !(c <= lead_max && s_lb > beat);
        if (!keep)
            pr.kept[pos] = kDropped;
        if (pr.bnd_count)
            pr.bnd_count[pos] = c, pr.bnd_score[pos] = s_lb;
        return keep;
    };
    const uint32_t nent = len - first;
    for (uint32_t u = wg; (uint64_t)u * 64u < nent; u += nwg) {
        const uint32_t e = first + u * 64u + (uint32_t)lane;
        const uint32_t pos = pr.sel[min(e, len - 1u)];
        const float4 *sh = reinterpret_cast<const float4 *>(a.models + (size_t)a.slots[pos] * kModelStride + kShadowOff);
        float4 rv[4];
#pragma unroll
        for (int k = 0; k < 4; ++k)
            rv[k] = sh[k];
        const uint32_t n = min(64u, nent - u * 64u);
        auto model_of_lane = [&](uint32_t j, float (&r)[16]) {
#pragma unroll
            for (int k = 0; k < 4; ++k) {
                r[4 * k + 0] = __builtin_bit_cast(float, __builtin_amdgcn_readlane(__builtin_bit_cast(int, rv[k].x), (int)j));
                r[4 * k + 1] = __builtin_bit_cast(float, __builtin_amdgcn_readlane(__builtin_bit_cast(int, rv[k].y), (int)j));
                r[4 * k + 2] = __builtin_bit_cast(float, __builtin_amdgcn_readlane(__builtin_bit_cast(int, rv[k].z), (int)j));
                r[4 * k + 3] = __builtin_bit_cast(float, __builtin_amdgcn_readlane(__builtin_bit_cast(int, rv[k].w), (int)j));
            }
        };
        uint32_t my_c = 0;
        uint64_t my_q = 0;
        for (uint32_t ch = (uint32_t)wave; ch < chunks; ch += (uint32_t)kWaves) {
            if (!resident)
                load_chunk(ch);
            for (uint32_t j = 0; j < n; ++j) {
                float r[16];
                model_of_lane(j, r);
                const float gt = pf_abs_bound_slack(r, pf.gx);
                uint32_t c = 0, q = 0;
#pragma unroll
                for (int p = 0; p + 1 < P; p += 2) {
                    const v2f Xp = {X[p], X[p + 1]}, Yp = {Y[p], Y[p + 1]}, Zp = {Z[p], Z[p + 1]};
                    const v2f xp = {x[p], x[p + 1]}, yp = {y[p], y[p + 1]}, w = {fw[p], fw[p + 1]};
                    const v2f z0 = pk_fma(bc(r[0]), Xp, pk_fma(bc(r[1]), Yp, pk_fma(bc(r[2]), Zp, bc(r[9]))));
                    const v2f z1 = pk_fma(bc(r[3]), Xp, pk_fma(bc(r[4]), Yp, pk_fma(bc(r[5]), Zp, bc(r[10]))));
                    const v2f z2 = pk_fma(bc(r[6]), Xp, pk_fma(bc(r[7]), Yp, pk_fma(bc(r[8]), Zp, bc(r[11]))));
                    const v2f a0 = pk_fma(-xp, z2, z0);
                    const v2f a1 = pk_fma(-yp, z2, z1);
                    const v2f W = w + bc(gt);
                    const v2f B = pk_fma(bc(pf.thr), z2, W);
#pragma unroll
                    for (int e2 = 0; e2 < 2; ++e2) {
                        const uint64_t out = vmask[p + e2] & (__builtin_amdgcn_ballot_w64(fmaxf(fabsf(a0[e2]), fabsf(a1[e2])) > B[e2]) |
                                                              __builtin_amdgcn_ballot_w64(z2[e2] < -W[e2]));
                        q += (uint32_t)__popcll(out);
                        c += (uint32_t)__popcll(vmask[p + e2] & ~out);
                    }
                }
                if constexpr (P & 1) {
                    constexpr int p = P - 1;
                    const uint64_t out = vmask[p] & __builtin_amdgcn_ballot_w64(pf_abs_outlier(r, gt, pf.thr, x[p], y[p], X[p], Y[p], Z[p], fw[p]));
                    q += (uint32_t)__popcll(out);
                    c += (uint32_t)__popcll(vmask[p] & ~out);
                }
                if ((uint32_t)lane == j)
                    my_c += c, my_q += q;
            }
        }
        s_c[wave][lane] = my_c;
        s_q[wave][lane] = my_q << 20;
        __syncthreads();
        bool open = false;
        if (wave == 0) {
            open = (uint32_t)lane < n && decide(pos);
            const uint64_t und = __builtin_amdgcn_ballot_w64(open);
            if (open)
                s_und[__builtin_amdgcn_mbcnt_hi((uint32_t)(und >> 32), __builtin_amdgcn_mbcnt_lo((uint32_t)und, 0u))] = (uint32_t)lane;
            if (lane == 0)
                s_nund = (uint32_t)__popcll(und);
        }
        __syncthreads();
        const uint32_t nund = (uint32_t)__builtin_amdgcn_readfirstlane((int)s_nund);
        if (nund) {
            my_c = 0, my_q = 0;
            for (uint32_t ch = (uint32_t)wave; ch < chunks; ch += (uint32_t)kWaves) {
                if (!resident)
                    load_chunk(ch);
                for (uint32_t k = 0; k < nund; ++k) {
                    const uint32_t j = (uint32_t)__builtin_amdgcn_readfirstlane((int)s_und[k]);
                    float r[16];
                    model_of_lane(j, r);
                    const float gt = pf_abs_bound_slack(r, pf.gx);
                    uint32_t c = 0, q = 0;
#pragma unroll
                    for (int p = 0; p < P; ++p) {
                        const float L = pf_abs_r2_lower(r, gt, x[p], y[p], X[p], Y[p], Z[p], fw[p]);
                        c += (uint32_t)__popcll(__builtin_amdgcn_ballot_w64(valid[p] && L < pf.thr2_up));
                        q += valid[p] ? pf_bound_quantum(L, pf.inv_thr2_dn) : 0u;
                    }
                    q = (uint32_t)__builtin_amdgcn_readlane((int)wave_scan_u32(q), 63);
                    if ((uint32_t)lane == j)
                        my_c += c, my_q += q;
                }
            }
            s_c[wave][lane] = my_c;
            s_q[wave][lane] = my_q;
            __syncthreads();
            if (open)
                (void)decide(pos);
        }
        __syncthreads();
    }
}
template <int P> __global__ __launch_bounds__(kBoundThreads) void k_score_bound(ScoreArgs a) { score_bound_body<P>(a, blockIdx.x, gridDim.x); }
__global__ __launch_bounds__(kBoundThreads) void k_score_bound_g(const GroupArgs *ga) {
    const GroupArgs &g = ga[blockIdx.z];
    if (!g.active || !g.use_mfma || !g.score.prune.st)
        return;
    score_bound_body<5>(globalised(g.score), blockIdx.x, gridDim.x);
}
__device__ __forceinline__ void prune_bound_body(const ScoreArgs &a) {
    __shared__ uint32_t wt[16];
    const PruneArgs &pr = a.prune;
    if (!pr.bound || pr.st->cstar >= pr.chunks)
        return;
    const uint32_t first = min(*a.num_hyp, pr.lead), len = pr.st->sel_len;
    const int lane = threadIdx.x & 63, wave = threadIdx.x >> 6;
    uint32_t base = 0;
    __syncthreads();
    for (uint32_t t0 = first; t0 < len; t0 += 1024u) {
        const uint32_t e = t0 + threadIdx.x;
        uint32_t keep = 0, p = 0;
        if (e < len) {
            p = pr.sel[e];
            keep = pr.kept[p] != kDropped ? 1u : 0u;
        }
        const uint32_t inc = wave_scan_u32(keep);
        if (lane == 63)
            wt[wave] = inc;
        __syncthreads();
        uint32_t at = base + inc - keep, tot = 0;
        for (int w = 0; w < 16; ++w) {
            at += w < wave ? wt[w] : 0u;
            tot += wt[w];
        }
        if (keep)
            pr.sel[at] = p;
        base += tot;
        __syncthreads();
    }
    if (threadIdx.x == 0)
        pr.st->sel_len = base;
}
__global__ __launch_bounds__(1024) void k_prune_bound(ScoreArgs a) { prune_bound_body(a); }
__global__ __launch_bounds__(1024) void k_prune_bound_g(const GroupArgs *ga) {
    const GroupArgs &g = ga[blockIdx.z];
    if (!g.active || !g.use_mfma || !g.score.prune.st)
        return;
    prune_bound_body(globalised(g.score));
}



template <int EST, int PG>
__device__ __forceinline__ void score_mfma2_body(const PointSet &pts, const uint4 *__restrict__ hypop,
                                                 const double *__restrict__ models, const uint32_t *__restrict__ slots,
                                                 const uint32_t *__restrict__ num_hyp_ptr, uint32_t hyp_capacity,
                                                 double thr2, const PrefilterArgs &pf, uint32_t *__restrict__ part_count,
                                                 double *__restrict__ part_score, uint32_t slice, uint32_t chunk,
                                                 uint32_t nslices) {
    static_assert(EST == EST_REL || EST == EST_FUND, "Sampson scores");
    constexpr int kWaves = kMfmaThreads / 64;
    constexpr int NPW = 32 * PG;
    constexpr int NBR = (EST == EST_REL) ? 6 : 1;
    __shared__ double s_pts[4][NPW];
    __shared__ double s_bear[NBR][(EST == EST_REL) ? NPW : 1];
    __shared__ uint16_t s_queue[kWaves][kMfmaQueueCap];
    __shared__ double s_acc_s[kWaves][64];
    __shared__ uint32_t s_acc_c[kWaves][64];
    __shared__ uint32_t s_next_unit;
    __shared__ uint4 s_bop[PG][3][64];
    const int lane = threadIdx.x & 63;
    const int wave = __builtin_amdgcn_readfirstlane((int)(threadIdx.x >> 6));
    const int col = lane & 31, half = lane >> 5;

    for (uint32_t j = threadIdx.x; j < (uint32_t)NPW; j += kMfmaThreads) {
        const uint32_t i = chunk * NPW + j;
        const uint32_t ic = i < pts.n ? i : 0u;
        const double a0 = pts.a[0][ic], a1 = pts.a[1][ic], b0 = pts.a[2][ic], b1 = pts.a[3][ic];
        s_pts[0][j] = a0, s_pts[1][j] = a1, s_pts[2][j] = b0, s_pts[3][j] = b1;
        if constexpr (EST == EST_REL) {
            const Vec3 u1 = bearing(a0, a1), u2 = bearing(b0, b1);
            s_bear[0][j] = u1.x, s_bear[1][j] = u1.y, s_bear[2][j] = u1.z;
            s_bear[3][j] = u2.x, s_bear[4][j] = u2.y, s_bear[5][j] = u2.z;
        }
    }
    uint32_t validbits = 0;
#pragma unroll
    for (int g = 0; g < PG; ++g)
        validbits |= (chunk * NPW + g * 32 + col < pts.n) ? (1u << (PG - 1 - g)) : 0u;
    for (uint32_t j = threadIdx.x; j < (uint32_t)NPW; j += kMfmaThreads) {
        const uint32_t i = chunk * NPW + j;
        const bool valid = i < pts.n;
        const uint32_t ic = valid ? i : 0u;
        Sampson16Operand o;
        pf16_sampson_point(pts.a[0][ic], pts.a[1][ic], pts.a[2][ic], pts.a[3][ic], valid, pf.t16, o);
#pragma unroll
        for (int b = 0; b < 6; ++b) {
            const uint16_t *h = b < 4 ? o.c + 8 * b : o.s + 8 * (b - 4);
            s_bop[j >> 5][b >> 1][(j & 31) + 32 * (b & 1)] =
                make_uint4((uint32_t)h[0] | ((uint32_t)h[1] << 16), (uint32_t)h[2] | ((uint32_t)h[3] << 16),
                           (uint32_t)h[4] | ((uint32_t)h[5] << 16), (uint32_t)h[6] | ((uint32_t)h[7] << 16));
        }
    }
    if (threadIdx.x == 0)
        s_next_unit = 0;
    __syncthreads();

    const uint32_t H = *as_uniform(num_hyp_ptr);
    const float t16 = pf.t16;
    uint16_t *const queue = s_queue[wave];
    double *const acc_s = s_acc_s[wave];
    uint32_t *const acc_c = s_acc_c[wave];
    const uint32_t waves_per_chunk = nslices * kWaves;
    auto request_ticket = [&]() -> uint32_t {
        uint32_t t = 0;
        if (lane == 0) {
            const uint32_t k = atomicAdd(&s_next_unit, 1u);
            t = slice * kWaves + (k % kWaves) + (k / kWaves) * waves_per_chunk;
        }
        return t;
    };
    uint32_t ticket = (uint32_t)__builtin_amdgcn_readfirstlane((int)request_ticket());
    uint32_t kb, gn;
    while (unit_of_ticket(ticket, H, waves_per_chunk, kb, gn)) {
        const uint32_t pending = request_ticket();
        const uint32_t unit_slots = slots[kb + min((uint32_t)lane, gn - 1u)];
        acc_s[lane] = 0.0;
        acc_c[lane] = 0;
        uint32_t qhead = 0, qtail = 0;

        auto drain = [&](uint32_t n) {
            __builtin_amdgcn_fence(__ATOMIC_ACQ_REL, "wavefront");
            const bool act = (uint32_t)lane < n;
            const uint32_t e = act ? (uint32_t)queue[(qhead + lane) & (kMfmaQueueCap - 1)] : 0xffffu;
            const uint32_t g = e >> 9, pi = act ? (e & 0x1ffu) : 0u;
            const double x0 = s_pts[0][pi], x1 = s_pts[1][pi], x2 = s_pts[2][pi], x3 = s_pts[3][pi];
            const double *Mp = models + (size_t)(uint32_t)__shfl((int)unit_slots, (int)(act ? g : 0u), 64) * kModelStride;
            double M[kModelDoubles];
#pragma unroll
            for (int i = 0; i < kModelDoubles; ++i)
                M[i] = Mp[i];
            double r2 = sampson_sq(M + kMatOff, x0, x1, x2, x3);
            bool in = r2 < thr2;
            if constexpr (EST == EST_REL) {
                if (in) {
                    Quat q;
                    q.w = M[0], q.x = M[1], q.y = M[2], q.z = M[3];
                    in = check_cheirality(q, v3(M[4], M[5], M[6]), v3(s_bear[0][pi], s_bear[1][pi], s_bear[2][pi]),
                                          v3(s_bear[3][pi], s_bear[4][pi], s_bear[5][pi]), 0.01);
                }
            }
// ... 1859 lines not shown
}

static uint32_t xcd_slices(uint32_t s) { return std::max<uint32_t>(1u, s); }

template <int E>
static hipError_t launch_score_est(const ScoreArgs &a, uint32_t slices, hipStream_t stream) {
    uint32_t chunks;
    int P;
    const PrefilterArgs pf = a.pf;
    const bool streaming = (a.shadow && a.compact64) || a.shadow16;
    score_shape(E, a.pts.n, streaming, a.shadow16 != nullptr, chunks, P);
    if constexpr (E == EST_REL || E == EST_FUND) {
        if (streaming && a.shadow16) {
            const uint32_t mslices = std::min<uint32_t>(slices * (uint32_t)kScoreThreads / (uint32_t)kMfmaThreads,
                                                        score_slice_limit(E, chunks, true));
            const dim3 mgrid(xcd_slices(mslices), chunks);
            const dim3 mblock(kMfmaThreads);
#define PL_M2_CASE(PP)                                                                                                 \
    case PP:                                                                                                           \
        k_score_mfma2<E, 2 * PP><<<mgrid, mblock, 0, stream>>>(a.pts, static_cast<const uint4 *>(a.shadow16), a.models, \
                                                              a.slots, a.num_hyp, a.hyp_capacity, a.thr2, pf,          \
                                                              a.part_count, a.part_score);                             \
        break;
            switch (P) {
                PL_M2_CASE(1)
                PL_M2_CASE(2)
                PL_M2_CASE(3)
                PL_M2_CASE(4)
                PL_M2_CASE(5)
                PL_M2_CASE(6)
            default:
                return hipErrorInvalidValue;
            }
#undef PL_M2_CASE
            return hipGetLastError();
        }
    }
    if constexpr (E == EST_HOM) {
        if (streaming && a.shadow16) {
            const dim3 mgrid(xcd_slices(slices * (uint32_t)kScoreThreads / (uint32_t)kMfmaThreads), chunks);
            const dim3 mblock(kMfmaThreads);
#define PL_MH_CASE(PP)                                                                                                 \
    case PP:                                                                                                           \
        k_score_mfmah<2 * PP><<<mgrid, mblock, 0, stream>>>(a.pts, static_cast<const uint4 *>(a.shadow16), a.models,    \
                                                          a.slots, a.num_hyp, a.hyp_capacity, a.thr2, pf, a.part_count, \
                                                          a.part_score);                                                \
        break;
            switch (P) {
                PL_MH_CASE(1)
                PL_MH_CASE(2)
                PL_MH_CASE(3)
                PL_MH_CASE(4)
                PL_MH_CASE(5)
            default:
                return hipErrorInvalidValue;
            }
#undef PL_MH_CASE
            return hipGetLastError();
        }
    }
    if constexpr (E == EST_ABS) {
        if (streaming && a.shadow16) {
            const uint32_t mslices = std::min<uint32_t>(slices * (uint32_t)kScoreThreads / (uint32_t)kMfmaThreads,
                                                        score_slice_limit(E, chunks, true));
            const dim3 mgrid(xcd_slices(mslices), chunks);
            const dim3 mblock(kMfmaThreads);
            if (!a.points16)
                return hipErrorInvalidValue;
#define PL_M_CASE(PP)                                                                                                  \
    case PP:                                                                                                           \
        k_score_mfma<2 * PP><<<mgrid, mblock, 0, stream>>>(a.pts, static_cast<const uint4 *>(a.shadow16),                \
                                                         static_cast<const uint4 *>(a.points16), a.models, a.slots,    \
                                                         a.num_hyp, a.hyp_capacity, a.thr2, a.part_count, a.part_score, \
                                                         a.tickets);                                                   \
        break;
            switch (P) {
                PL_M_CASE(1)
                PL_M_CASE(2)
                PL_M_CASE(3)
                PL_M_CASE(4)
                PL_M_CASE(5)
            default:
                return hipErrorInvalidValue;
            }
#undef PL_M_CASE
            return hipGetLastError();
        }
    }
    if (streaming) {
        const dim3 qgrid(std::max<uint32_t>(1u, slices * (uint32_t)kScoreThreads / (uint32_t)kQueueThreads), chunks);
        const dim3 qblock(kQueueThreads);
#define PL_Q_CASE(PP)                                                                                                  \
    case PP:                                                                                                           \
        k_score_queue<E, PP><<<qgrid, qblock, 0, stream>>>(a.pts, a.shadow, a.compact64, a.num_hyp, a.hyp_capacity,      \
                                                         a.thr2, pf, a.part_count, a.part_score, a.tickets);           \
        break;
        switch (P) {
            PL_Q_CASE(1)
            PL_Q_CASE(2)
            PL_Q_CASE(3)
            PL_Q_CASE(4)
            PL_Q_CASE(5)
            PL_Q_CASE(6)
        default:
            return hipErrorInvalidValue;
        }
#undef PL_Q_CASE
        return hipGetLastError();
    }
    return hipErrorInvalidValue;
}

hipError_t launch_score_seq(int est, const SeqScoreArgs &a, hipStream_t stream) {
    if (a.cap == 0)
        return hipSuccess;
    const dim3 grid(std::min<uint32_t>(a.cap, 128u)), block(kSeqThreads);
    PL_DISPATCH_EST_0TO5(est, k_score_seq<E><<<grid, block, 0, stream>>>(a));
    return hipGetLastError();
}
int tangent_score_chunk() { return kTangentChunk; }
int radial1d_score_chunk() { return kRadialChunk; }
hipError_t launch_prune_lead(const ScoreArgs &a, hipStream_t stream) {
    k_prune_lead<<<dim3(1), dim3(256), 0, stream>>>(a);
    return hipGetLastError();
}
hipError_t launch_prune_select(const ScoreArgs &a, hipStream_t stream) {
    const uint32_t nb = std::max<uint32_t>(1u, (a.hyp_capacity + 1023u) / 1024u);
    k_prune_flags<<<dim3(nb), dim3(1024), 0, stream>>>(a);
    k_prune_list<<<dim3(nb), dim3(1024), 0, stream>>>(a);
    return hipGetLastError();
}
hipError_t launch_group_prune_lead(const GroupArgs *args, const GroupDims &d, hipStream_t stream) {
    k_prune_lead_g<<<dim3(1, 1, d.G), dim3(256), 0, stream>>>(args);
    return hipGetLastError();
}
hipError_t launch_group_prune_select(const GroupArgs *args, const GroupDims &d, hipStream_t stream) {
    const uint32_t nb = std::max<uint32_t>(1u, (d.max_hcap + 1023u) / 1024u);
    k_prune_flags_g<<<dim3(nb, 1, d.G), dim3(1024), 0, stream>>>(args);
    k_prune_list_g<<<dim3(nb, 1, d.G), dim3(1024), 0, stream>>>(args);
    return hipGetLastError();
}
template <int PG> static hipError_t launch_score_pruned_pg(const ScoreArgs &a, dim3 grid, hipStream_t stream) {
    const dim3 block(kMfmaThreads);
    const dim3 lead_grid(pruned_slices<kScoreLead>(grid.x), grid.y), sel_grid(pruned_slices<kScoreSel>(grid.x), grid.y);
    k_score_mfma_pr<PG, kScoreLead><<<lead_grid, block, 0, stream>>>(a);
    hipError_t e = launch_prune_lead(a, stream);
    if (e != hipSuccess)
        return e;
    k_score_mfma_pr<PG, kScoreCount><<<grid, block, 0, stream>>>(a);
    e = launch_prune_select(a, stream);
    if (e != hipSuccess)
        return e;
    if (a.prune.bound) {
        k_score_bound<PG / 2><<<dim3(kBoundGroups), dim3(kBoundThreads), 0, stream>>>(a);
        k_prune_bound<<<dim3(1), dim3(1024), 0, stream>>>(a);
    }
    k_score_mfma_pr<PG, kScoreSel><<<sel_grid, block, 0, stream>>>(a);
    return hipGetLastError();
}
static hipError_t pruned_grid(const ScoreArgs &a, uint32_t slices, dim3 &grid, int &P) {
    uint32_t chunks;
    score_shape(EST_ABS, a.pts.n, true, true, chunks, P);
    if (!a.shadow16 || !a.points16 || !a.prune.st || a.prune.chunks != chunks || a.prune.chunk_points != 64u * (uint32_t)P)
        return hipErrorInvalidValue;
    const uint32_t mslices = std::min<uint32_t>(slices * (uint32_t)kScoreThreads / (uint32_t)kMfmaThreads,
                                                score_slice_limit(EST_ABS, chunks, true));
    grid = dim3(xcd_slices(mslices), chunks);
    return (P == 4 || P == 5) ? hipSuccess : hipErrorInvalidValue;
}
hipError_t launch_score_pruned(const ScoreArgs &a, uint32_t slices, hipStream_t stream) {
    dim3 grid;
    int P;
    const hipError_t e = pruned_grid(a, slices, grid, P);
    if (e != hipSuccess)
        return e;
    return P == 4 ? launch_score_pruned_pg<8>(a, grid, stream) : launch_score_pruned_pg<10>(a, grid, stream);
}
hipError_t launch_score_count(const ScoreArgs &a, uint32_t slices, hipStream_t stream) {
    dim3 grid;
    int P;
    const hipError_t e = pruned_grid(a, slices, grid, P);
    if (e != hipSuccess)
        return e;
    if (P == 4)
        k_score_mfma_pr<8, kScoreCountAll><<<grid, dim3(kMfmaThreads), 0, stream>>>(a);
    else
        k_score_mfma_pr<10, kScoreCountAll><<<grid, dim3(kMfmaThreads), 0, stream>>>(a);
    return hipGetLastError();
}
hipError_t launch_prune_label(const ScoreArgs &a, hipStream_t stream) {
    k_prune_label<<<dim3(std::max<uint32_t>(1u, (a.hyp_capacity + 255u) / 256u)), dim3(256), 0, stream>>>(a);
    return hipGetLastError();
}

hipError_t launch_score(int est, const ScoreArgs &a, uint32_t slices, hipStream_t stream) {
    if (est == EST_RAD1D) {
        if (!a.shadow || !a.compact64)
            return hipErrorInvalidValue;
        const uint32_t chunks = score_chunks(est, a.pts.n, true, false);
        const dim3 qgrid(std::max<uint32_t>(1u, slices * (uint32_t)kScoreThreads / (uint32_t)kQueueThreads), chunks);
        k_score_radial1d<<<qgrid, dim3(kQueueThreads), 0, stream>>>(a.pts, a.shadow, a.compact64, a.num_hyp, a.hyp_capacity, a.thr2, a.pf,
                                                                    a.part_count, a.part_score);
        return hipGetLastError();
    }
    if (est == EST_RELT) {
        if (!a.shadow || !a.compact64)
            return hipErrorInvalidValue;
        const uint32_t chunks = score_chunks(est, a.pts.n, true, false);
        const dim3 qgrid(std::max<uint32_t>(1u, slices * (uint32_t)kScoreThreads / (uint32_t)kQueueThreads), chunks);
        k_score_tangent<<<qgrid, dim3(kQueueThreads), 0, stream>>>(a.pts, a.shadow, a.compact64, a.num_hyp, a.hyp_capacity, a.thr2, a.pf,
                                                                   a.part_count, a.part_score);
        return hipGetLastError();
    }
    PL_DISPATCH_EST(est, return launch_score_est<E>(a, slices, stream));
    return hipSuccess;
}


hipError_t launch_lm(int est, const PointSet &pts, LMTask *tasks, uint32_t num_tasks, hipStream_t stream) {
    const size_t want = sizeof(double) * point_doubles(est) * (size_t)pts.n;
    return launch_lm_tasks(est, tasks, num_tasks, want <= 128 * 1024 ? pts.n : 0u, stream);
}
static std::atomic<int> g_lm_mode{-1};
void set_lm_mode(int mode) { g_lm_mode.store((mode == 1 || mode == 2) ? mode : 0, std::memory_order_release); }
int get_lm_mode() {
    int m = g_lm_mode.load(std::memory_order_acquire);
    if (m < 0) {
        const char *e = std::getenv("POSELIB_AMD_LM_ORDERED");
        m = (e && e[0] == '1') ? 1 : (e && e[0] == '2') ? 2 : 0;
        g_lm_mode.store(m, std::memory_order_release);
    }
    return m;
}
static thread_local int tl_lm_force_ordered = 0;
void set_lm_force_ordered(int on) { tl_lm_force_ordered = on; }
bool lm_sums_ordered(int est) {
    if (tl_lm_force_ordered)
        return true;
    const int m = get_lm_mode();
    return est != EST_RELT && (m == 1 || (m == 0 && est == EST_FUND));
}
#ifdef PL_LM_PROFILE
extern "C" int pl_debug_lm_profile(unsigned long long *out16, int reset) {
    if (hipMemcpyFromSymbol(out16, HIP_SYMBOL(g_lm_prof), sizeof(unsigned long long) * 16) != hipSuccess)
        return -1;
    if (reset) {
        unsigned long long z[16] = {0};
        if (hipMemcpyToSymbol(HIP_SYMBOL(g_lm_prof), z, sizeof(z)) != hipSuccess)
            return -1;
    }
    return 0;
}
#endif
hipError_t launch_lm_tasks(int est, LMTask *tasks, uint32_t num_tasks, uint32_t max_points, hipStream_t stream) {
    if (num_tasks == 0)
        return hipSuccess;
    if (est < 0 || est > EST_RAD1D)
        return hipErrorInvalidValue;
    const int ordered = lm_sums_ordered(est) ? 1 : 0;
    static std::atomic<int> dyn_limit[2][6] = {{{-1}, {-1}, {-1}, {-1}, {-1}, {-1}}, {{-1}, {-1}, {-1}, {-1}, {-1}, {-1}}};
    int limit = dyn_limit[ordered][est].load(std::memory_order_acquire);
    if (limit < 0) {
        hipFuncAttributes fa;
        hipError_t e = hipSuccess;
        if (ordered) {
            PL_DISPATCH_EST_0123_5(est, e = hipFuncGetAttributes(&fa, reinterpret_cast<const void *>(&k_lm_ordered<E>)));
        } else {
            PL_DISPATCH_EST_0TO5(est, e = hipFuncGetAttributes(&fa, reinterpret_cast<const void *>(&k_lm<E>)));
        }
        if (e != hipSuccess)
            return e;
        limit = std::max<int>(0, 160 * 1024 - (int)fa.sharedSizeBytes - 1024);
        limit = std::min<int>(limit, 128 * 1024);
        if (limit > 48 * 1024) {
            if (ordered) {
                PL_DISPATCH_EST_0123_5(est, e = hipFuncSetAttribute(reinterpret_cast<const void *>(&k_lm_ordered<E>),
                                                             hipFuncAttributeMaxDynamicSharedMemorySize, limit));
            } else {
                PL_DISPATCH_EST_0TO5(est, e = hipFuncSetAttribute(reinterpret_cast<const void *>(&k_lm<E>),
                                                              hipFuncAttributeMaxDynamicSharedMemorySize, limit));
            }
            if (e != hipSuccess)
                return e;
        }
        dyn_limit[ordered][est].store(limit, std::memory_order_release);
    }
    const size_t want = sizeof(double) * point_doubles(est) * (size_t)max_points;
    const size_t bytes = want <= (size_t)limit ? want : 0;
    if (ordered) {
        PL_DISPATCH_EST_0123_5(est, k_lm_ordered<E><<<dim3(num_tasks), dim3(kLMThreads), bytes, stream>>>(tasks, (uint32_t)bytes));
    } else {
        PL_DISPATCH_EST_0TO5(est, k_lm<E><<<dim3(num_tasks), dim3(kLMThreads), bytes, stream>>>(tasks, (uint32_t)bytes));
    }
    return hipGetLastError();
}

__global__ void k_task_records(int est, const LMTask *tasks, const double *records_in, double *records_out,
                               uint32_t num_tasks, LMTask *host_tasks) {
    const uint32_t j = blockIdx.x * blockDim.x + threadIdx.x;
    if (j >= num_tasks)
        return;
    if (host_tasks) {
        for (int i = 0; i < kParamDoubles; ++i)
            host_tasks[j].params[i] = tasks[j].params[i];
        host_tasks[j].iterations = tasks[j].iterations;
        host_tasks[j].skipped = tasks[j].skipped;
        host_tasks[j].cost = tasks[j].cost;
        host_tasks[j].initial_cost = tasks[j].initial_cost;
    }
    double *out = records_out + (size_t)j * kModelStride;
    if (tasks[j].skipped) {
        for (int i = 0; i < kModelStride; ++i)
            out[i] = records_in[(size_t)j * kModelStride + i];
    } else {
        record_from_lm_params(est, tasks[j].params, out);
    }
}
__global__ void k_select_record(const double *score_refined, double incumbent_score, const double *rec_refined,
                                const double *rec_incumbent, double *out) {
    const double *src = (*score_refined < incumbent_score) ? rec_refined : rec_incumbent;
    if (threadIdx.x < kModelStride)
        out[threadIdx.x] = src[threadIdx.x];
}
__global__ void k_select_record_g(const SelectArgs *arr) {
    const SelectArgs a = globalised(arr[blockIdx.z]);
    if (!a.out)
        return;
    const double *src = (*a.score_refined < a.incumbent_score) ? a.rec_refined : a.rec_incumbent;
    if (threadIdx.x < kModelStride)
        a.out[threadIdx.x] = src[threadIdx.x];
    if (threadIdx.x == 63 && a.fetch_src)
        *a.fetch_dst = *a.fetch_src;
    if (threadIdx.x == 62 && a.count_out)
        *a.count_out = (*a.score_refined < a.incumbent_score) ? *a.count_refined : a.count_incumbent;
}
hipError_t launch_group_select(const SelectArgs *args, uint32_t G, hipStream_t stream) {
    if (G == 0)
        return hipSuccess;
    k_select_record_g<<<dim3(1, 1, G), dim3(64), 0, stream>>>(args);
    return hipGetLastError();
}
hipError_t launch_group_mask(int est, const MaskArgs *args, uint32_t G, uint32_t max_n, hipStream_t stream) {
    if (G == 0 || max_n == 0)
        return hipSuccess;
    const dim3 grid((max_n + 255) / 256, 1, G), block(256);
    PL_DISPATCH_EST(est, k_mask_g<E><<<grid, block, 0, stream>>>(args));
    return hipGetLastError();
}
hipError_t launch_group_score_seq(int est, const SeqScoreArgs *args, uint32_t G, uint32_t max_cap, hipStream_t stream) {
    if (G == 0 || max_cap == 0)
        return hipSuccess;
    const dim3 grid(std::min<uint32_t>(max_cap, 128u), 1, G), block(kSeqThreads);
    PL_DISPATCH_EST(est, k_score_seq_g<E><<<grid, block, 0, stream>>>(args));
    return hipGetLastError();
}

int group_points_per_lane(int est) { return (est == EST_REL || est == EST_FUND) ? 6 : 5; }

template <int E> static hipError_t launch_group_score_est(const GroupArgs *args, const GroupDims &d, hipStream_t stream) {
    const dim3 grid(std::max<uint32_t>(1u, d.max_slices), std::max<uint32_t>(1u, d.max_chunks), d.G);
    if constexpr (E == EST_ABS) {
        if (d.any_mfma && d.any_prune) {
            const dim3 lead_grid(pruned_slices<kScoreLead>(grid.x), grid.y, grid.z), sel_grid(pruned_slices<kScoreSel>(grid.x), grid.y, grid.z);
            k_score_mfma_pr_g<10, kScoreLead><<<lead_grid, dim3(kMfmaThreads), 0, stream>>>(args);
            hipError_t e = launch_group_prune_lead(args, d, stream);
            if (e != hipSuccess)
                return e;
            k_score_mfma_pr_g<10, kScoreCount><<<grid, dim3(kMfmaThreads), 0, stream>>>(args);
            e = launch_group_prune_select(args, d, stream);
            if (e != hipSuccess)
                return e;
            if (d.any_bound) {
                k_score_bound_g<<<dim3(kBoundGroups, 1, d.G), dim3(kBoundThreads), 0, stream>>>(args);
                k_prune_bound_g<<<dim3(1, 1, d.G), dim3(1024), 0, stream>>>(args);
            }
            k_score_mfma_pr_g<10, kScoreSel><<<sel_grid, dim3(kMfmaThreads), 0, stream>>>(args);
        } else if (d.any_mfma)
            k_score_mfma_g<10><<<grid, dim3(kMfmaThreads), 0, stream>>>(args);
        if (d.any_queue)
            k_score_queue_g<EST_ABS, 5><<<grid, dim3(kQueueThreads), 0, stream>>>(args);
    } else if constexpr (E == EST_HOM) {
        if (d.any_mfma)
            k_score_mfmah_g<10><<<grid, dim3(kMfmaThreads), 0, stream>>>(args);
        if (d.any_queue)
            k_score_queue_g<EST_HOM, 5><<<grid, dim3(kQueueThreads), 0, stream>>>(args);
    } else {
        if (d.any_mfma)
            k_score_mfma2_g<E, 2 * group_mfma2_points_per_lane(E)><<<grid, dim3(kMfmaThreads), 0, stream>>>(args);
        if (d.any_queue)
            k_score_queue_g<E, 6><<<grid, dim3(kQueueThreads), 0, stream>>>(args);
    }
    return hipGetLastError();
}

hipError_t launch_group_score_count(const GroupArgs *args, const GroupDims &d, hipStream_t stream) {
    const dim3 grid(std::max<uint32_t>(1u, d.max_slices), std::max<uint32_t>(1u, d.max_chunks), d.G);
    k_score_mfma_pr_g<10, kScoreCountAll><<<grid, dim3(kMfmaThreads), 0, stream>>>(args);
    return hipGetLastError();
}
hipError_t launch_group_score(int est, const GroupArgs *args, const GroupDims &d, hipStream_t stream) {
    if (d.G == 0)
        return hipSuccess;
    hipError_t e = hipSuccess;
    PL_DISPATCH_EST(est, e = launch_group_score_est<E>(args, d, stream));
    return e;
}

hipError_t launch_group_generate(int est, const GroupArgs *args, uint32_t max_B, uint32_t G, hipStream_t stream) {
    if (G == 0 || max_B == 0)
        return hipSuccess;
    if (est == EST_REL)
        return launch_group_generate_rel(args, max_B, G, stream);
    const dim3 ggrid((max_B + 63) / 64, 1, G), gblock(64);
    PL_DISPATCH_EST(est, k_generate_g<E><<<ggrid, gblock, 0, stream>>>(args));
    return hipGetLastError();
}

hipError_t launch_group_batch(int est, const GroupArgs *args, const GroupDims &d, hipStream_t stream, hipEvent_t ev0,
                              hipEvent_t ev1) {
    if (d.G == 0)
        return hipSuccess;
    hipError_t e = launch_group_positions(sample_size(est), args, d, stream);
    if (e != hipSuccess)
        return e;
    e = launch_group_generate(est, args, d.max_B, d.G, stream);
    if (e != hipSuccess)
        return e;
    e = launch_group_compact(args, d, stream);
    if (e != hipSuccess)
        return e;
    if (ev0 && (e = hipEventRecord(ev0, stream)) != hipSuccess)
        return e;
    e = launch_group_score(est, args, d, stream);
    if (e != hipSuccess)
        return e;
    if (ev1 && (e = hipEventRecord(ev1, stream)) != hipSuccess)
        return e;
    e = launch_group_finalize_records(args, d, stream);
    if (e != hipSuccess)
        return e;
    const uint32_t per_problem = std::max<uint32_t>(16u, std::min<uint32_t>(128u, 4096u / std::max<uint32_t>(1u, d.G)));
    const dim3 sgrid(per_problem, 1, d.G), sblock(kSeqThreads);
    PL_DISPATCH_EST(est, k_score_seq_gb<E><<<sgrid, sblock, 0, stream>>>(args));
    return hipGetLastError();
}

hipError_t launch_task_records(int est, const LMTask *tasks, const double *records_in, double *records_out,
                               uint32_t num_tasks, LMTask *host_tasks, hipStream_t stream) {
    if (num_tasks == 0)
        return hipSuccess;
    k_task_records<<<dim3((num_tasks + 63) / 64), dim3(64), 0, stream>>>(est, tasks, records_in, records_out, num_tasks,
                                                                         host_tasks);
    return hipGetLastError();
}
hipError_t launch_select_record(const double *score_refined, double incumbent_score, const double *rec_refined,
                                const double *rec_incumbent, double *out, hipStream_t stream) {
    k_select_record<<<dim3(1), dim3(64), 0, stream>>>(score_refined, incumbent_score, rec_refined, rec_incumbent, out);
    return hipGetLastError();
}

size_t lm2_state_bytes(uint32_t num_tasks) { return sizeof(LM2State) * 2 * (size_t)num_tasks; }
size_t lm2_partial_bytes(uint32_t num_tasks, uint32_t slices) { return sizeof(double) * 2 * (size_t)num_tasks * slices * 48; }
hipError_t launch_lm2(int est, const PointSet &pts, LMTask *tasks, uint32_t num_tasks, uint32_t slices,
                      uint32_t max_iterations, bool loss_changes, void *states, double *partials, hipStream_t stream) {
    if (num_tasks == 0)
        return hipSuccess;
    if (est == EST_REL)
        return hipErrorInvalidValue;
    const dim3 grid(slices, num_tasks), block(kLM2Threads);
    const uint32_t launches = (loss_changes ? 2u : 1u) * max_iterations + 2;
    for (uint32_t l = 0; l < launches; ++l) {
        switch (est) {
        case EST_ABS:
            k_lm2<EST_ABS><<<grid, block, 0, stream>>>(pts, tasks, static_cast<LM2State *>(states), partials, (int)(l & 1), l == 0);
            break;
        case EST_FUND:
            k_lm2<EST_FUND><<<grid, block, 0, stream>>>(pts, tasks, static_cast<LM2State *>(states), partials, (int)(l & 1), l == 0);
            break;
        default:
            k_lm2<EST_HOM><<<grid, block, 0, stream>>>(pts, tasks, static_cast<LM2State *>(states), partials, (int)(l & 1), l == 0);
            break;
        }
    }
    return hipGetLastError();
}

hipError_t launch_mask(int est, const PointSet &pts, const double *model, double thr2, uint8_t *mask,
                       uint8_t *host_mask, hipStream_t stream, const MaskDest *dst) {
    if (pts.n == 0)
        return hipSuccess;
    const dim3 grid((pts.n + 255) / 256), block(256);
    const MaskDest none = {nullptr, 0, nullptr};
    const MaskDest d = dst ? *dst : none;
    PL_DISPATCH_EST_0TO5(est, k_mask<E><<<grid, block, 0, stream>>>(pts, model, thr2, mask, host_mask, d));
    return hipGetLastError();
}

}
```

Before: 1.374 billion hypotheses/s.

## Pre-count selected hypotheses on tensor cores before bound pass, skip dead lanes

Adds a new kScoreCountSel MFMA pass that runs before the bound kernel. It computes exact per-chunk inlier counts for the selected hypotheses from chunk cstar onward and writes them into part_count. The bound kernel now first marks which lanes are still live, then runs the costly outlier-bound sweep only for those. It also loads its chunk lazily, and a debug API exposes the per-chunk columns. This is meant to cut bound-kernel work spent on hypotheses that are already settled, at the cost of an extra kernel launch and more synchronisation.

```diff
diff --git a/include/poselib_amd.h b/include/poselib_amd.h
--- a/include/poselib_amd.h
+++ b/include/poselib_amd.h
@@ -299,6 +299,9 @@
                              uint32_t *idle_changed, uint32_t *guard_changed);
 int pl_debug_score_bounded(int route, pl_debug_prune_member *members, size_t num_members, uint32_t *const *bound_counts,
                            double *const *bound_scores, uint8_t *const *tiers, uint32_t *idle_changed, uint32_t *guard_changed);
+int pl_debug_score_bounded_columns(int route, pl_debug_prune_member *members, size_t num_members, uint32_t *const *bound_counts,
+                                   double *const *bound_scores, uint8_t *const *tiers, uint32_t *const *columns, uint32_t *idle_changed,
+                                   uint32_t *guard_changed);
 int pl_debug_score_prune_gate(int kind, uint32_t n_points, uint32_t iterations);
 int pl_debug_lm_route(int kind, uint32_t n_points, uint64_t max_iterations, uint32_t *slices);
 typedef struct pl_debug_sampler_shape_info {
diff --git a/poselib_amd/_lib.py b/poselib_amd/_lib.py
--- a/poselib_amd/_lib.py
+++ b/poselib_amd/_lib.py
@@ -236,6 +236,8 @@
         "pl_debug_score_survivors": (cint, [cint, P(DebugPruneMember), sz, P(C.c_void_p), P(C.c_uint32), P(C.c_uint32)]),
         "pl_debug_score_bounded": (cint, [cint, P(DebugPruneMember), sz, P(C.c_void_p), P(C.c_void_p), P(C.c_void_p), P(C.c_uint32),
                                            P(C.c_uint32)]),
+        "pl_debug_score_bounded_columns": (cint, [cint, P(DebugPruneMember), sz, P(C.c_void_p), P(C.c_void_p), P(C.c_void_p), P(C.c_void_p),
+                                                   P(C.c_uint32), P(C.c_uint32)]),
         "pl_debug_score_prune_gate": (cint, [cint, C.c_uint32, C.c_uint32]),
         "pl_debug_lm_route": (cint, [cint, C.c_uint32, u64, P(C.c_uint32)]),
         "pl_debug_sampler_shape": (cint, [cint, u64, C.c_uint32, u64, P(DebugSamplerShape)]),
@@ -280,7 +282,7 @@
     "pl_abi_version", "pl_problem_create_tangent", "pl_debug_inlier_mask", "pl_debug_tangent_chunk",
     "pl_p5lp_radial", "pl_debug_radial1d_chunk", "pl_debug_radial1d_generate", "pl_debug_group_slices", "pl_debug_generate",
     "pl_debug_score_shape", "pl_debug_score_stream_ex", "pl_debug_score_pruned", "pl_debug_score_survivors", "pl_debug_score_prune_gate",
-    "pl_debug_score_bounded", "pl_debug_lm_route",
+    "pl_debug_score_bounded", "pl_debug_score_bounded_columns", "pl_debug_lm_route",
     "pl_estimate_absolute_pose_dev", "pl_estimate_relative_pose_dev", "pl_estimate_fundamental_dev", "pl_estimate_homography_dev",
     "pl_problem_create_dev", "pl_problem_create_tangent_dev", "pl_debug_check_device_points", "pl_debug_point_stats_dev",
     "pl_debug_sampler_shape", "pl_debug_sample_positions", "pl_estimate_batch_dev", "pl_debug_point_stats_group_dev",
diff --git a/poselib_amd/api.py b/poselib_amd/api.py
--- a/poselib_amd/api.py
+++ b/poselib_amd/api.py
@@ -859,9 +859,9 @@
     return out, idle.value, guard.value
 
 
-def score_bounded(members, route=0):
+def score_bounded(members, route=0, columns=False):
     arr = (L.DebugPruneMember * max(len(members), 1))()
-    bcs, bss, trs = ((C.c_void_p * max(len(members), 1))() for _ in range(3))
+    bcs, bss, trs, cls = ((C.c_void_p * max(len(members), 1))() for _ in range(4))
     keep = []
     cap = 4096
     for i, (problem, models, max_error, init_max, init_min) in enumerate(members):
@@ -877,16 +877,27 @@
         arr[i] = L.DebugPruneMember(problem._h, _ptr(flat), n, float(max_error), float(init_min), int(init_max), cap, _ptr(cnt),
                                     _ptr(sc), _ptr(kp), _ptr(cand))
         bcs[i], bss[i], trs[i] = bc.ctypes.data, bs.ctypes.data, tr.ctypes.data
+        if columns:
+            cl = np.zeros((score_shape(problem.kind, problem.n, True, route == 2)[0], max(n, 1)), dtype=np.uint32)
+            keep[-1] += (cl,)
+            cls[i] = cl.ctypes.data
     idle, guard = C.c_uint32(0), C.c_uint32(0)
-    L.check(L.lib().pl_debug_score_bounded(int(route), arr, C.c_size_t(len(members)), bcs, bss, trs, C.byref(idle), C.byref(guard)))
+    if columns:
+        L.check(L.lib().pl_debug_score_bounded_columns(int(route), arr, C.c_size_t(len(members)), bcs, bss, trs, cls, C.byref(idle),
+                                                       C.byref(guard)))
+    else:
+        L.check(L.lib().pl_debug_score_bounded(int(route), arr, C.c_size_t(len(members)), bcs, bss, trs, C.byref(idle), C.byref(guard)))
     out = []
-    for i, (n, _, cnt, sc, kp, cand, bc, bs, tr) in enumerate(keep):
+    for i, (n, _, cnt, sc, kp, cand, bc, bs, tr, *cl) in enumerate(keep):
         a = arr[i]
         out.append({"counts": cnt[:n], "scores": sc[:n], "kept": kp[:n].astype(bool), "cand": cand[:min(a.num_cand, cap)].copy(),
                     "num_cand": a.num_cand, "cstar": a.cstar, "chunks": a.chunks, "chunk_points": a.chunk_points, "lead": a.lead,
                     "lead_max": a.lead_max, "lead_min": a.lead_min, "num_live": a.num_live, "num_selected": a.num_selected,
                     "num_preselected": a.num_preselected, "slices": a.slices, "bound_counts": bc[:n], "bound_scores": bs[:n],
                     "tiers": tr[:n]})
+        if cl:
+            assert a.chunks == cl[0].shape[0], (a.chunks, cl[0].shape)
+            out[-1]["columns"] = cl[0][:, :n]
     return out, idle.value, guard.value
 
 
diff --git a/poselib_amd/csrc/driver.cc b/poselib_amd/csrc/driver.cc
--- a/poselib_amd/csrc/driver.cc
+++ b/poselib_amd/csrc/driver.cc
@@ -2629,6 +2629,7 @@
     uint32_t *const *bound_counts;
     double *const *bound_scores;
     uint8_t *const *tiers;
+    uint32_t *const *columns = nullptr;
 };
 int debug_score_pruned(int route, pl_debug_prune_member *m, size_t count, uint32_t *idle_changed, uint32_t *const *survivors = nullptr,
                        uint32_t *guard_changed = nullptr, const DebugBoundedOut *bounded = nullptr) {
@@ -2838,6 +2839,8 @@
                 bounded->bound_counts[i][k] = has ? bcount[i][p] : 0xffffffffu;
                 bounded->bound_scores[i][k] = has ? bscore[i][p] : std::numeric_limits<double>::quiet_NaN();
                 bounded->tiers[i][k] = !live ? 3 : kept[i][p] == kKept ? 0 : has ? 2 : 1;
+                for (uint32_t ch = 0; bounded->columns && ch < chunks; ++ch)
+                    bounded->columns[i][(size_t)ch * H + k] = live ? part[i][(size_t)ch * hcap + p] : 0u;
             }
         }
         const bool split = st[i].cstar < chunks;
@@ -2894,6 +2897,21 @@
         if (!bound_counts[i] || !bound_scores[i] || !tiers[i])
             return fail(PL_ERR_INVALID, "pl_debug_score_bounded: a member without an output array");
     const DebugBoundedOut out{bound_counts, bound_scores, tiers};
+    return debug_score_pruned(route, members, num_members, idle_changed, nullptr, guard_changed, &out);
+}
+int pl_debug_score_bounded_columns(int route, pl_debug_prune_member *members, size_t num_members, uint32_t *const *bound_counts,
+                                   double *const *bound_scores, uint8_t *const *tiers, uint32_t *const *columns, uint32_t *idle_changed,
+                                   uint32_t *guard_changed) {
+    if (idle_changed)
+        *idle_changed = 0;
+    if (guard_changed)
+        *guard_changed = 0;
+    if (!bound_counts || !bound_scores || !tiers || !columns)
+        return fail(PL_ERR_INVALID, "pl_debug_score_bounded_columns: output arrays missing");
+    for (size_t i = 0; i < num_members; ++i)
+        if (!bound_counts[i] || !bound_scores[i] || !tiers[i] || !columns[i])
+            return fail(PL_ERR_INVALID, "pl_debug_score_bounded_columns: a member without an output array");
+    const DebugBoundedOut out{bound_counts, bound_scores, tiers, columns};
     return debug_score_pruned(route, members, num_members, idle_changed, nullptr, guard_changed, &out);
 }
 int pl_debug_score_prune_gate(int kind, uint32_t n_points, uint32_t iterations) {
diff --git a/poselib_amd/csrc/kernels.hip b/poselib_amd/csrc/kernels.hip
--- a/poselib_amd/csrc/kernels.hip
+++ b/poselib_amd/csrc/kernels.hip
@@ -1219,7 +1219,7 @@
     return 16u * PG - n;
 }
 
-constexpr int kScoreAll = 0, kScoreLead = 1, kScoreSel = 2, kScoreCount = 3, kScoreCountAll = 4;
+constexpr int kScoreAll = 0, kScoreLead = 1, kScoreSel = 2, kScoreCount = 3, kScoreCountAll = 4, kScoreCountSel = 5;
 template <int PG, int MODE = kScoreAll>
 __device__ __forceinline__ void score_mfma_body(const PointSet &pts, const uint4 *__restrict__ shadow16,
                                                 const uint4 *__restrict__ points16,
@@ -1378,11 +1378,11 @@
     }
 }
 
-template <int PG>
+template <int PG, bool SEL = false>
 __device__ __forceinline__ void score_count_body(uint32_t n_points, const uint4 *__restrict__ shadow16, const uint4 *__restrict__ points16,
                                                  const uint32_t *__restrict__ num_hyp_ptr, uint32_t hyp_capacity,
                                                  uint32_t *__restrict__ survivors, uint32_t slice, uint32_t chunk, uint32_t nslices,
-                                                 uint32_t first) {
+                                                 uint32_t first, const uint32_t *__restrict__ sel = nullptr) {
     constexpr int kWaves = kMfmaThreads / 64;
     constexpr int NPW = 32 * PG;
     __shared__ uint4 s_b[1 + kAbs16Dirs][PG][32];
@@ -1423,8 +1423,11 @@
     while (unit_of_ticket<32u>(ticket, H, waves_per_chunk, kb, gn)) {
         const uint32_t pending = request_ticket();
         const uint32_t ngroups32 = (gn + 31u) / 32u;
+        uint32_t next_pos = 0;
         auto load_a = [&](uint32_t hg, uint4 (&A)[kAbs16Dirs]) {
             const uint4 *row = shadow16 + (size_t)min(first + kb + 32u * hg + (uint32_t)col, Hall - 1u) * 4;
+            if constexpr (SEL)
+                row = shadow16 + (size_t)(next_pos = sel[min(first + kb + 32u * hg + (uint32_t)col, Hall - 1u)]) * 4;
 #pragma unroll
             for (int d = 0; d < kAbs16Dirs; ++d)
                 A[d] = row[half ? 3 : d];
@@ -1436,6 +1439,7 @@
 #pragma unroll
             for (int d = 0; d < kAbs16Dirs; ++d)
                 __builtin_memcpy(&Aop[d], &Araw[d], 16);
+            [[maybe_unused]] const uint32_t pos = next_pos;
             if (hg + 1 < ngroups32)
                 load_a(hg + 1, Araw);
             const uint32_t mine = abs16_tile_count_t<PG>(Aop, s_b, col, half);
@@ -1443,7 +1447,10 @@
             uint32_t total = both[0] + both[1];
             if (pad)
                 total = max(total, pad) - pad;
-            if (half == 0 && 32u * hg + (uint32_t)col < gn)
+            if constexpr (SEL) {
+                if (half == 0 && 32u * hg + (uint32_t)col < gn)
+                    survivors[(size_t)chunk * hyp_capacity + pos] = total;
+            } else if (half == 0 && 32u * hg + (uint32_t)col < gn)
                 survivors[(size_t)chunk * hyp_capacity + first + kb + 32u * hg + (uint32_t)col] = total;
         }
         ticket = (uint32_t)__builtin_amdgcn_readfirstlane((int)pending);
@@ -1477,10 +1484,11 @@
                         a.num_hyp, a.hyp_capacity, a.thr2, a.part_count, a.part_score, slice, chunk, g.slices);
 }
 template <int MODE> __host__ __device__ constexpr uint32_t pruned_slices(uint32_t slices) {
-    return MODE == kScoreLead ? (slices < 2u ? slices : 2u) : MODE == kScoreSel ? (slices + 3u) / 4u : slices;
+    return MODE == kScoreLead ? (slices < 2u ? slices : 2u) : (MODE == kScoreSel || MODE == kScoreCountSel) ? (slices + 3u) / 4u : slices;
 }
 template <int PG, int MODE> __device__ __forceinline__ void score_mfma_pruned(const ScoreArgs &a, uint32_t slice, uint32_t chunk, uint32_t nslices) {
-    static_assert(MODE == kScoreLead || MODE == kScoreSel || MODE == kScoreCount || MODE == kScoreCountAll, "the plain launch is k_score_mfma's");
+    static_assert(MODE == kScoreLead || MODE == kScoreSel || MODE == kScoreCount || MODE == kScoreCountAll || MODE == kScoreCountSel,
+                  "the plain launch is k_score_mfma's");
     const PruneArgs &pr = a.prune;
     if (!pr.st && MODE != kScoreSel)
         return;
@@ -1493,6 +1501,14 @@
             return;
         score_count_body<PG>(a.pts.n, static_cast<const uint4 *>(a.shadow16), static_cast<const uint4 *>(a.points16), a.num_hyp,
                              a.hyp_capacity, a.part_count, slice, chunk, nslices, pr.lead);
+    } else if constexpr (MODE == kScoreCountSel) {
+        if (!pr.bound)
+            return;
+        const uint32_t cstar = *as_uniform(&pr.st->cstar);
+        if (cstar >= pr.chunks || chunk < cstar)
+            return;
+        score_count_body<PG, true>(a.pts.n, static_cast<const uint4 *>(a.shadow16), static_cast<const uint4 *>(a.points16), &pr.st->sel_len,
+                                   a.hyp_capacity, a.part_count, slice, chunk, nslices, min(*as_uniform(a.num_hyp), pr.lead), pr.sel);
     } else {
         const uint32_t *len = MODE == kScoreSel && pr.st ? &pr.st->sel_len : a.num_hyp;
         score_mfma_body<PG, MODE>(a.pts, static_cast<const uint4 *>(a.shadow16), static_cast<const uint4 *>(a.points16), a.models, a.slots,
@@ -1669,8 +1685,9 @@
     constexpr uint32_t NPW = 64u * P;
     __shared__ uint32_t s_c[kWaves][64];
     __shared__ uint64_t s_q[kWaves][64];
+    __shared__ uint32_t s_liv[64];
     __shared__ uint32_t s_und[64];
-    __shared__ uint32_t s_nund;
+    __shared__ uint32_t s_nliv, s_nund;
     const PruneArgs &pr = a.prune;
     if (!pr.st || !pr.bound || *as_uniform(&pr.st->cstar) >= pr.chunks)
         return;
@@ -1698,17 +1715,10 @@
             fw[p] = pf_point_abs(Xd, Yd, Zd, pf.gx);
         }
     };
-    load_chunk(min((uint32_t)wave, chunks - 1u));
+    bool loaded = false;
     const uint32_t lead_max = pr.st->lead_max;
     const double beat = pr.st->lead_min * (1.0 + kPruneScoreMargin);
-    auto decide = [&](uint32_t pos) -> bool {
-        uint32_t c = 0;
-        uint64_t q = 0;
-#pragma unroll
-        for (int w = 0; w < kWaves; ++w) {
-            c += s_c[w][lane];
-            q += s_q[w][lane];
-        }
+    auto decide = [&](uint32_t pos, uint32_t c, uint64_t q) -> bool {
         const double qd = (double)q * 9.5367431640625e-07;
         double s_lb = a.thr2 * qd;
         if (fma(a.thr2, qd, -s_lb) < 0.0)
@@ -1720,105 +1730,136 @@
             pr.bnd_count[pos] = c, pr.bnd_score[pos] = s_lb;
         return keep;
     };
+    auto decide_partials = [&](uint32_t pos) -> bool {
+        uint32_t c = 0;
+        uint64_t q = 0;
+#pragma unroll
+        for (int w = 0; w < kWaves; ++w) {
+            c += s_c[w][lane];
+            q += s_q[w][lane];
+        }
+        return decide(pos, c, q);
+    };
     const uint32_t nent = len - first;
     for (uint32_t u = wg; (uint64_t)u * 64u < nent; u += nwg) {
         const uint32_t e = first + u * 64u + (uint32_t)lane;
         const uint32_t pos = pr.sel[min(e, len - 1u)];
-        const float4 *sh = reinterpret_cast<const float4 *>(a.models + (size_t)a.slots[pos] * kModelStride + kShadowOff);
-        float4 rv[4];
-#pragma unroll
-        for (int k = 0; k < 4; ++k)
-            rv[k] = sh[k];
         const uint32_t n = min(64u, nent - u * 64u);
-        auto model_of_lane = [&](uint32_t j, float (&r)[16]) {
-#pragma unroll
-            for (int k = 0; k < 4; ++k) {
-                r[4 * k + 0] = __builtin_bit_cast(float, __builtin_amdgcn_readlane(__builtin_bit_cast(int, rv[k].x), (int)j));
-                r[4 * k + 1] = __builtin_bit_cast(float, __builtin_amdgcn_readlane(__builtin_bit_cast(int, rv[k].y), (int)j));
-                r[4 * k + 2] = __builtin_bit_cast(float, __builtin_amdgcn_readlane(__builtin_bit_cast(int, rv[k].z), (int)j));
-                r[4 * k + 3] = __builtin_bit_cast(float, __builtin_amdgcn_readlane(__builtin_bit_cast(int, rv[k].w), (int)j));
-            }
-        };
-        uint32_t my_c = 0;
-        uint64_t my_q = 0;
-        for (uint32_t ch = (uint32_t)wave; ch < chunks; ch += (uint32_t)kWaves) {
-            if (!resident)
-                load_chunk(ch);
-            for (uint32_t j = 0; j < n; ++j) {
-                float r[16];
-                model_of_lane(j, r);
-                const float gt = pf_abs_bound_slack(r, pf.gx);
-                uint32_t c = 0, q = 0;
-#pragma unroll
-                for (int p = 0; p + 1 < P; p += 2) {
-                    const v2f Xp = {X[p], X[p + 1]}, Yp = {Y[p], Y[p + 1]}, Zp = {Z[p], Z[p + 1]};
-                    const v2f xp = {x[p], x[p + 1]}, yp = {y[p], y[p + 1]}, w = {fw[p], fw[p + 1]};
-                    const v2f z0 = pk_fma(bc(r[0]), Xp, pk_fma(bc(r[1]), Yp, pk_fma(bc(r[2]), Zp, bc(r[9]))));
-                    const v2f z1 = pk_fma(bc(r[3]), Xp, pk_fma(bc(r[4]), Yp, pk_fma(bc(r[5]), Zp, bc(r[10]))));
-                    const v2f z2 = pk_fma(bc(r[6]), Xp, pk_fma(bc(r[7]), Yp, pk_fma(bc(r[8]), Zp, bc(r[11]))));
-                    const v2f a0 = pk_fma(-xp, z2, z0);
-                    const v2f a1 = pk_fma(-yp, z2, z1);
-                    const v2f W = w + bc(gt);
-                    const v2f B = pk_fma(bc(pf.thr), z2, W);
-#pragma unroll
-                    for (int e2 = 0; e2 < 2; ++e2) {
-                        const uint64_t out = vmask[p + e2] & (__builtin_amdgcn_ballot_w64(fmaxf(fabsf(a0[e2]), fabsf(a1[e2])) > B[e2]) |
-                                                              __builtin_amdgcn_ballot_w64(z2[e2] < -W[e2]));
-                        q += (uint32_t)__popcll(out);
-                        c += (uint32_t)__popcll(vmask[p + e2] & ~out);
-                    }
+        bool live = false;
+        if (wave == 0) {
+            if ((uint32_t)lane < n) {
+                uint32_t c = 0;
+                for (uint32_t ch = 0; ch < chunks; ++ch)
+                    c += a.part_count[(size_t)ch * a.hyp_capacity + pos];
+                c = min(c, a.pts.n);
+                live = decide(pos, c, (uint64_t)(a.pts.n - c) << 20);
+            }
+            const uint64_t liv = __builtin_amdgcn_ballot_w64(live);
+            if (live)
+                s_liv[__builtin_amdgcn_mbcnt_hi((uint32_t)(liv >> 32), __builtin_amdgcn_mbcnt_lo((uint32_t)liv, 0u))] = (uint32_t)lane;
+            if (lane == 0)
+                s_nliv = (uint32_t)__popcll(liv);
+        }
+        __syncthreads();
+        const uint32_t nliv = (uint32_t)__builtin_amdgcn_readfirstlane((int)s_nliv);
+        if (nliv) {
+            const float4 *sh = reinterpret_cast<const float4 *>(a.models + (size_t)a.slots[pos] * kModelStride + kShadowOff);
+            float4 rv[4];
+#pragma unroll
+            for (int k = 0; k < 4; ++k)
+                rv[k] = sh[k];
+            auto model_of_lane = [&](uint32_t j, float (&r)[16]) {
+#pragma unroll
+                for (int k = 0; k < 4; ++k) {
+                    r[4 * k + 0] = __builtin_bit_cast(float, __builtin_amdgcn_readlane(__builtin_bit_cast(int, rv[k].x), (int)j));
+                    r[4 * k + 1] = __builtin_bit_cast(float, __builtin_amdgcn_readlane(__builtin_bit_cast(int, rv[k].y), (int)j));
+                    r[4 * k + 2] = __builtin_bit_cast(float, __builtin_amdgcn_readlane(__builtin_bit_cast(int, rv[k].z), (int)j));
+                    r[4 * k + 3] = __builtin_bit_cast(float, __builtin_amdgcn_readlane(__builtin_bit_cast(int, rv[k].w), (int)j));
                 }
-                if constexpr (P & 1) {
-                    constexpr int p = P - 1;
-                    const uint64_t out = vmask[p] & __builtin_amdgcn_ballot_w64(pf_abs_outlier(r, gt, pf.thr, x[p], y[p], X[p], Y[p], Z[p], fw[p]));
-                    q += (uint32_t)__popcll(out);
-                    c += (uint32_t)__popcll(vmask[p] & ~out);
-                }
-                if ((uint32_t)lane == j)
-                    my_c += c, my_q += q;
-            }
-        }
-        s_c[wave][lane] = my_c;
-        s_q[wave][lane] = my_q << 20;
-        __syncthreads();
-        bool open = false;
-        if (wave == 0) {
-            open = (uint32_t)lane < n && decide(pos);
-            const uint64_t und = __builtin_amdgcn_ballot_w64(open);
-            if (open)
-                s_und[__builtin_amdgcn_mbcnt_hi((uint32_t)(und >> 32), __builtin_amdgcn_mbcnt_lo((uint32_t)und, 0u))] = (uint32_t)lane;
-            if (lane == 0)
-                s_nund = (uint32_t)__popcll(und);
-        }
-        __syncthreads();
-        const uint32_t nund = (uint32_t)__builtin_amdgcn_readfirstlane((int)s_nund);
-        if (nund) {
-            my_c = 0, my_q = 0;
+            };
+            uint32_t my_c = 0;
+            uint64_t my_q = 0;
             for (uint32_t ch = (uint32_t)wave; ch < chunks; ch += (uint32_t)kWaves) {
-                if (!resident)
+                if (!resident || !loaded)
                     load_chunk(ch);
-                for (uint32_t k = 0; k < nund; ++k) {
-                    const uint32_t j = (uint32_t)__builtin_amdgcn_readfirstlane((int)s_und[k]);
+                for (uint32_t k = 0; k < nliv; ++k) {
+                    const uint32_t j = (uint32_t)__builtin_amdgcn_readfirstlane((int)s_liv[k]);
                     float r[16];
                     model_of_lane(j, r);
                     const float gt = pf_abs_bound_slack(r, pf.gx);
                     uint32_t c = 0, q = 0;
 #pragma unroll
-                    for (int p = 0; p < P; ++p) {
-                        const float L = pf_abs_r2_lower(r, gt, x[p], y[p], X[p], Y[p], Z[p], fw[p]);
-                        c += (uint32_t)__popcll(__builtin_amdgcn_ballot_w64(valid[p] && L < pf.thr2_up));
-                        q += valid[p] ? pf_bound_quantum(L, pf.inv_thr2_dn) : 0u;
+                    for (int p = 0; p + 1 < P; p += 2) {
+                        const v2f Xp = {X[p], X[p + 1]}, Yp = {Y[p], Y[p + 1]}, Zp = {Z[p], Z[p + 1]};
+                        const v2f xp = {x[p], x[p + 1]}, yp = {y[p], y[p + 1]}, w = {fw[p], fw[p + 1]};
+                        const v2f z0 = pk_fma(bc(r[0]), Xp, pk_fma(bc(r[1]), Yp, pk_fma(bc(r[2]), Zp, bc(r[9]))));
+                        const v2f z1 = pk_fma(bc(r[3]), Xp, pk_fma(bc(r[4]), Yp, pk_fma(bc(r[5]), Zp, bc(r[10]))));
+                        const v2f z2 = pk_fma(bc(r[6]), Xp, pk_fma(bc(r[7]), Yp, pk_fma(bc(r[8]), Zp, bc(r[11]))));
+                        const v2f a0 = pk_fma(-xp, z2, z0);
+                        const v2f a1 = pk_fma(-yp, z2, z1);
+                        const v2f W = w + bc(gt);
+                        const v2f B = pk_fma(bc(pf.thr), z2, W);
+#pragma unroll
+                        for (int e2 = 0; e2 < 2; ++e2) {
+                            const uint64_t out = vmask[p + e2] & (__builtin_amdgcn_ballot_w64(fmaxf(fabsf(a0[e2]), fabsf(a1[e2])) > B[e2]) |
+                                                                  __builtin_amdgcn_ballot_w64(z2[e2] < -W[e2]));
+                            q += (uint32_t)__popcll(out);
+                            c += (uint32_t)__popcll(vmask[p + e2] & ~out);
+                        }
                     }
-                    q = (uint32_t)__builtin_amdgcn_readlane((int)wave_scan_u32(q), 63);
+                    if constexpr (P & 1) {
+                        constexpr int p = P - 1;
+                        const uint64_t out = vmask[p] & __builtin_amdgcn_ballot_w64(pf_abs_outlier(r, gt, pf.thr, x[p], y[p], X[p], Y[p], Z[p], fw[p]));
+                        q += (uint32_t)__popcll(out);
+                        c += (uint32_t)__popcll(vmask[p] & ~out);
+                    }
                     if ((uint32_t)lane == j)
                         my_c += c, my_q += q;
                 }
             }
+            loaded = true;
             s_c[wave][lane] = my_c;
-            s_q[wave][lane] = my_q;
+            s_q[wave][lane] = my_q << 20;
             __syncthreads();
-            if (open)
-                (void)decide(pos);
+            bool open = false;
+            if (wave == 0) {
+                open = live && decide_partials(pos);
+                const uint64_t und = __builtin_amdgcn_ballot_w64(open);
+                if (open)
+                    s_und[__builtin_amdgcn_mbcnt_hi((uint32_t)(und >> 32), __builtin_amdgcn_mbcnt_lo((uint32_t)und, 0u))] = (uint32_t)lane;
+                if (lane == 0)
+                    s_nund = (uint32_t)__popcll(und);
+            }
+            __syncthreads();
+            const uint32_t nund = (uint32_t)__builtin_amdgcn_readfirstlane((int)s_nund);
+            if (nund) {
+                my_c = 0, my_q = 0;
+                for (uint32_t ch = (uint32_t)wave; ch < chunks; ch += (uint32_t)kWaves) {
+                    if (!resident)
+                        load_chunk(ch);
+                    for (uint32_t k = 0; k < nund; ++k) {
+                        const uint32_t j = (uint32_t)__builtin_amdgcn_readfirstlane((int)s_und[k]);
+                        float r[16];
+                        model_of_lane(j, r);
+                        const float gt = pf_abs_bound_slack(r, pf.gx);
+                        uint32_t c = 0, q = 0;
+#pragma unroll
+                        for (int p = 0; p < P; ++p) {
+                            const float L = pf_abs_r2_lower(r, gt, x[p], y[p], X[p], Y[p], Z[p], fw[p]);
+                            c += (uint32_t)__popcll(__builtin_amdgcn_ballot_w64(valid[p] && L < pf.thr2_up));
+                            q += valid[p] ? pf_bound_quantum(L, pf.inv_thr2_dn) : 0u;
+                        }
+                        q = (uint32_t)__builtin_amdgcn_readlane((int)wave_scan_u32(q), 63);
+                        if ((uint32_t)lane == j)
+                            my_c += c, my_q += q;
+                    }
+                }
+                s_c[wave][lane] = my_c;
+                s_q[wave][lane] = my_q;
+                __syncthreads();
+                if (open)
+                    (void)decide_partials(pos);
+            }
         }
         __syncthreads();
     }
@@ -3984,6 +4025,7 @@
     if (e != hipSuccess)
         return e;
     if (a.prune.bound) {
+        k_score_mfma_pr<PG, kScoreCountSel><<<sel_grid, block, 0, stream>>>(a);
         k_score_bound<PG / 2><<<dim3(kBoundGroups), dim3(kBoundThreads), 0, stream>>>(a);
         k_prune_bound<<<dim3(1), dim3(1024), 0, stream>>>(a);
     }
@@ -4203,6 +4245,7 @@
             if (e != hipSuccess)
                 return e;
             if (d.any_bound) {
+                k_score_mfma_pr_g<10, kScoreCountSel><<<sel_grid, dim3(kMfmaThreads), 0, stream>>>(args);
                 k_score_bound_g<<<dim3(kBoundGroups, 1, d.G), dim3(kBoundThreads), 0, stream>>>(args);
                 k_prune_bound_g<<<dim3(1, 1, d.G), dim3(1024), 0, stream>>>(args);
             }
```

Measured after the change: 1.409 billion hypotheses/s, median of 6. 2.5% higher.
